# dwofk/fast-depth

Hardware: NVIDIA H100
Metric: depth-maps/sec @224x224 b64 (higher is better)
Workload: dtype f16

## Files before the change

### fastdepth_b200/csrc/fd_api.cu

```cuda
#include <algorithm>
#include <cstring>
#include <functional>
#include <string>
#include <vector>

#include "fd_block_plan.h"
#include "fd_conv_plan.h"
#include "fd_common.cuh"

namespace fd {

BlockPlanOut block_tc_debug_plan(int ksize, int stride, int h_out, int w_out, int n, int c_in, int c_out, int head);
ConvPlanOut conv_tc_debug_plan(int kind, int ksize, int h_out, int w_out, int n, int c_in, int c_out, int n_sms);
ConvPlanOut pw_tf32x3_debug_plan(int h_out, int w_out, int n, int c_in, int c_out, int upsample, int n_sms);

static thread_local std::string g_last_error;
void set_error(const std::string& msg) { g_last_error = msg; }
int fail(int code, const std::string& msg) {
    g_last_error = msg;
    return code;
}

int launch_stem(int dtype, const void* x, void* out, const float* w, const float* scale, const float* bias,
                const StageGeom& g, cudaStream_t st);
int launch_dw(int dtype, const BlockArgs& a, cudaStream_t st);
int launch_pw(int dtype, const BlockArgs& a, cudaStream_t st);
int launch_conv(int dtype, const void* in, const void* w, void* out, const float* scale, const float* bias, const StageGeom& g,
                cudaStream_t st);
int launch_convt(int dtype, int kind, const void* in, const void* w, void* out, const float* scale, const float* bias,
                 const StageGeom& g, cudaStream_t st);
int launch_head(int dtype, const void* in, void* out, const float* w, float scale, float bias, long long m_total, int c,
                int in_pitch, int h, int wd, int up, int act, cudaStream_t st);
int launch_metrics(int dtype, const void* pred, const float* target, int n, int hw, double* sums, cudaStream_t st);
int launch_nyu_val_gather(int dtype, const uint8_t* rgb, const float* depth, const int* rows, const int* cols, int n, int h_in,
                          int w_in, int oh, int ow, void* x, float* t, cudaStream_t st);
struct BlockTcPlan;
bool block_tc_supported(int dtype, const StageGeom& g, bool head_fused);
int block_tc_prepare(int dtype, const BlockArgs& a, const float* head_w, float head_scale, float head_bias, int head_act,
                     void* head_out, bool tma_epilogue, const TcLaunchOpts& opts, BlockTcPlan** out);
int block_tc_launch(BlockTcPlan* p, cudaStream_t st, void* head_out);
void block_tc_destroy(BlockTcPlan* p);
const char* block_tc_name(BlockTcPlan* p);
int block_tc_trace(BlockTcPlan* bp, cudaStream_t st, void* head_out, unsigned long long* out_host, int* rows, int* cols);
struct ChainTcPlan;
bool chain_tc_supported(int dtype, const StageGeom* g, int n_layers);
int chain_tc_prepare(int dtype, const BlockArgs* layers, int n_layers, const TcLaunchOpts& opts, ChainTcPlan** out);
int chain_tc_launch(ChainTcPlan* cp, cudaStream_t st);
void chain_tc_destroy(ChainTcPlan* cp);
const char* chain_tc_name(ChainTcPlan* cp);
int chain_tc_trace(ChainTcPlan* cp, cudaStream_t st, unsigned long long* out_host, int* rows, int* cols);
struct StemTcPlan;
bool stem_tc_supported(int dtype, const StageGeom& g);
int stem_tc_prepare(int dtype, const StageGeom& g, const float* w27_dev, const float* scale_dev, const float* bias_dev, void* out,
                    const TcLaunchOpts& opts, StemTcPlan** res);
int stem_tc_launch(StemTcPlan* sp, const void* x, cudaStream_t st);
void stem_tc_destroy(StemTcPlan* sp);
const char* stem_tc_name(StemTcPlan* sp);
struct ConvTcPlan;
bool conv_tc_supported(int dtype, const StageGeom& g, int kind);
int conv_tc_prepare(int dtype, int kind, const StageGeom& g, const void* in, const void* w, const float* scale_dev,
                    const float* bias_dev, void* out, const TcLaunchOpts& opts, ConvTcPlan** res);
int conv_tc_launch(ConvTcPlan* cp, cudaStream_t st);
void conv_tc_destroy(ConvTcPlan* cp);
const char* conv_tc_name(ConvTcPlan* cp);
bool pw_tf32x3_supported(const StageGeom& g);
int pw_tf32x3_prepare(const StageGeom& g, const void* mid, const float* w, const float* scale_dev, const float* bias_dev,
                      void* out, int out_pitch, int reduce, const TcLaunchOpts& opts, ConvTcPlan** res);

static size_t dtype_size(int dtype) { return dtype == FD_F32 ? 4 : 2; }
static bool is_phased(int kind) { return kind == FD_STAGE_DECONV || kind == FD_STAGE_UPCONV; }
static bool is_conv(int kind) { return kind == FD_STAGE_CONV || is_phased(kind); }

struct Stage {
    fd_stage_desc d{};
    StageGeom g{};
    int out_h = 0, out_w = 0;
    void* out = nullptr;
    void* out_eff = nullptr;
    void* out_alloc = nullptr;
    int out_c = 0;
    int out_pitch = 0;
    int concat_src = -1;
    void* mid = nullptr;
    float* dw_w = nullptr;
    float* dw_scale = nullptr;
    float* dw_bias = nullptr;
    void* pw_w = nullptr;
    float* pw_w_f32 = nullptr;
    float* pw_scale = nullptr;
    float* pw_bias = nullptr;
    float head_scale = 0.f, head_bias = 0.f;
    bool have_weights = false;
    BlockTcPlan* tc = nullptr;
    StemTcPlan* stc = nullptr;
    ConvTcPlan* ctc = nullptr;
    ChainTcPlan* chain = nullptr;
    int chained = 0;
};

struct Step {
    int stage;
    std::string name;
    double alg_bytes, macs;
    double dw_macs = 0.0;
    std::function<int(cudaStream_t, const void*, void*)> run;
};

}

using namespace fd;

struct fd_plan {
    int n = 0, h = 0, w = 0, dtype = 0, device = 0, n_sms = 132;
    std::vector<Stage> stages;
    std::vector<Step> steps;
    bool steps_valid = false;
    int opt_path = 1, opt_fold_head = 1, opt_graph = 1, opt_tma_epilogue = 1, opt_inplace_skip = 1, opt_pdl = 0, opt_wait_sleep_ns = 0;
    int opt_chain = 1;
    int opt_cluster = 1;
    int opt_tf32x3 = 0;
    size_t workspace_bytes = 0;
    struct PipeSlot { void* x = nullptr; void* y = nullptr; cudaEvent_t up = nullptr, done = nullptr, down = nullptr; bool busy = false; };
    PipeSlot pipe[3];
    cudaStream_t pipe_h2d = nullptr, pipe_run = nullptr, pipe_d2h = nullptr;
    unsigned long long pipe_next = 0;
    void* stage_x = nullptr;
    void* stage_y = nullptr;
    cudaEvent_t last_done = nullptr;
    cudaStream_t last_stream = nullptr;
    bool last_stream_set = false;
    void* l2_flush = nullptr;
    size_t l2_flush_bytes = 0;
    struct GraphEntry { const void* x; void* y; cudaGraphExec_t exec; unsigned long long stamp; };
    std::vector<GraphEntry> graphs;
    unsigned long long graph_clock = 0;
    int graph_misses = 0;
};
static const size_t kMaxGraphs = 8;

namespace fd {

struct DeviceGuard {
    int prev = -1;
    bool ok = true;
    explicit DeviceGuard(int dev) {
        if (cudaGetDevice(&prev) != cudaSuccess) { ok = false; return; }
        if (prev != dev && cudaSetDevice(dev) != cudaSuccess) ok = false;
    }
    ~DeviceGuard() {
        if (prev >= 0) cudaSetDevice(prev);
    }
};

static int dev_alloc(fd_plan* p, void** ptr, size_t bytes) {
    bytes = (bytes + 255) & ~size_t(255);
    FD_CUDA_OK(cudaMalloc(ptr, bytes));
    FD_CUDA_OK(cudaMemset(*ptr, 0, bytes));
    p->workspace_bytes += bytes;
    return FD_OK;
}

static void invalidate(fd_plan* p) {
    p->steps_valid = false;
    p->steps.clear();
    for (auto& g : p->graphs) cudaGraphExecDestroy(g.exec);
    p->graphs.clear();
    for (auto& s : p->stages) {
        if (s.tc) { block_tc_destroy(s.tc); s.tc = nullptr; }
        if (s.stc) { stem_tc_destroy(s.stc); s.stc = nullptr; }
        if (s.ctc) { conv_tc_destroy(s.ctc); s.ctc = nullptr; }
        if (s.chain) { chain_tc_destroy(s.chain); s.chain = nullptr; }
        s.chained = 0;
    }
}

static int upload_as_dtype(int dtype, const float* host, size_t count, void* dev) {
    if (dtype == FD_F32) {
        FD_CUDA_OK(cudaMemcpy(dev, host, count * 4, cudaMemcpyHostToDevice));
    } else if (dtype == FD_F16) {
        std::vector<__half> tmp(count);
        for (size_t i = 0; i < count; ++i) tmp[i] = __float2half_rn(host[i]);
        FD_CUDA_OK(cudaMemcpy(dev, tmp.data(), count * 2, cudaMemcpyHostToDevice));
    } else {
        std::vector<__nv_bfloat16> tmp(count);
        for (size_t i = 0; i < count; ++i) tmp[i] = __float2bfloat16_rn(host[i]);
        FD_CUDA_OK(cudaMemcpy(dev, tmp.data(), count * 2, cudaMemcpyHostToDevice));
    }
    return FD_OK;
}

static int build_steps(fd_plan* p) {
    invalidate(p);
    const int ns = (int)p->stages.size();
    const double es = (double)dtype_size(p->dtype);
    for (auto& s : p->stages)
        if (!s.have_weights) return fail(FD_ERR_STATE, "fd_plan_set_stage_weights was not called for every stage");

    TcLaunchOpts lopts;
    lopts.pdl = p->opt_pdl; lopts.sleep_ns = p->opt_wait_sleep_ns; lopts.n_sms = p->n_sms; lopts.cluster = p->opt_cluster;
    Stage& head = p->stages[ns - 1];
    Stage& last = p->stages[ns - 2];
    const bool fold = p->opt_fold_head && (last.d.kind == FD_STAGE_DWPW || last.d.kind == FD_STAGE_CONV) && last.d.upsample &&
                      last.d.skip_src < 0;
    bool head_fused = false;

    for (int i = 0; i < ns; ++i) {
        Stage& s = p->stages[i];
        const void* in = i > 0 ? p->stages[i - 1].out_eff : nullptr;
        s.out_eff = s.out;
        s.g.in_pitch = i > 0 ? p->stages[i - 1].out_pitch : 0;
        s.g.out_pitch = s.out_pitch;
        s.g.skip_pitch = (s.d.skip_src >= 0 && !s.d.skip_mode) ? p->stages[s.d.skip_src].out_pitch : s.out_pitch;
        if (s.d.kind == FD_STAGE_STEM) {
            Step st;
            st.stage = i;
            st.name = "stem_kernel";
            st.macs = (double)s.g.n * s.g.h_out * s.g.w_out * s.g.c_out * 27.0;
            st.alg_bytes = ((double)s.g.n * 3 * s.g.h_in * s.g.w_in + (double)s.g.n * s.g.h_out * s.g.w_out * s.g.c_out) * es +
                           29.0 * s.g.c_out * 4;
            Stage* sp = &s;
            const int dtype = p->dtype;
            if (p->opt_path == 1 && stem_tc_supported(dtype, s.g)) {
                int rc = stem_tc_prepare(dtype, s.g, s.pw_w_f32, s.pw_scale, s.pw_bias, s.out, lopts, &s.stc);
                if (rc != FD_OK) return rc;
                st.name = stem_tc_name(s.stc);
                StemTcPlan* stc = s.stc;
                st.run = [stc](cudaStream_t stream, const void* x, void*) { return stem_tc_launch(stc, x, stream); };
            } else {
                st.run = [sp, dtype](cudaStream_t stream, const void* x, void*) {
                    return launch_stem(dtype, x, sp->out, sp->pw_w_f32, sp->pw_scale, sp->pw_bias, sp->g, stream);
                };
            }
            p->steps.push_back(st);
        } else if (is_conv(s.d.kind)) {
            StageGeom g = s.g;
            if (fold && &s == &last) g.upsample = 0;
            const int kind = s.d.kind;
            const double px_in = (double)g.n * g.h_in * g.w_in, px_out = (double)g.n * g.h_out * g.w_out;
            const double kk = (double)g.ksize * g.ksize;
            Step st;
            st.stage = i;
            st.macs = px_out * g.c_in * g.c_out * kk;
            st.dw_macs = 0.0;
            st.alg_bytes = (px_in * g.c_in + px_out * (g.upsample || is_phased(kind) ? 4.0 : 1.0) * g.c_out) * es +
                           kk * g.c_in * g.c_out * es + 2.0 * g.c_out * 4;
            const int dtype = p->dtype;
            if (p->opt_path == 1 && conv_tc_supported(dtype, g, kind)) {
                int rc = conv_tc_prepare(dtype, kind, g, in, s.pw_w, s.pw_scale, s.pw_bias, s.out, lopts, &s.ctc);
                if (rc != FD_OK) return rc;
                st.name = conv_tc_name(s.ctc);
                ConvTcPlan* ctc = s.ctc;
                st.run = [ctc](cudaStream_t stream, const void*, void*) { return conv_tc_launch(ctc, stream); };
            } else if (kind == FD_STAGE_CONV) {
                char nm[64];
                snprintf(nm, sizeof(nm), "conv_kernel<k%d>", g.ksize);
                st.name = nm;
                Stage* sp = &s;
                st.run = [sp, in, g, dtype](cudaStream_t stream, const void*, void*) {
                    return launch_conv(dtype, in, sp->pw_w, sp->out, sp->pw_scale, sp->pw_bias, g, stream);
                };
            } else {
                char nm[64];
                snprintf(nm, sizeof(nm), "convt_kernel<%s%d>", kind == FD_STAGE_DECONV ? "deconv" : "upconv", g.ksize);
                st.name = nm;
                Stage* sp = &s;
                st.run = [sp, in, g, dtype, kind](cudaStream_t stream, const void*, void*) {
                    return launch_convt(dtype, kind, in, sp->pw_w, sp->out, sp->pw_scale, sp->pw_bias, g, stream);
                };
            }
            p->steps.push_back(st);
        } else if (s.d.kind == FD_STAGE_DWPW && s.chained) {
            continue;
        } else if (s.d.kind == FD_STAGE_DWPW) {
            if (p->opt_path == 1 && p->opt_chain) {
                std::vector<BlockArgs> run;
                std::vector<StageGeom> geoms;
                int j = i;
                for (; j < ns - 1 && (int)run.size() < 8; ++j) {
                    Stage& t = p->stages[j];
                    if (t.d.kind != FD_STAGE_DWPW || t.d.ksize != 3 || t.d.stride != 1 || t.d.upsample || t.d.skip_src >= 0) break;
                    if (j > i && p->stages[j - 1].concat_src >= 0) break;
                    bool is_skip_source = false;
                    for (int k2 = j + 1; k2 < ns; ++k2) if (p->stages[k2].d.skip_src == j) is_skip_source = true;
                    BlockArgs b{};
                    b.g = t.g;
                    b.g.in_pitch = j > 0 ? p->stages[j - 1].out_pitch : 0;
                    b.g.out_pitch = t.out_pitch;
                    b.in = j > 0 ? p->stages[j - 1].out_eff : nullptr;
                    b.out = t.out;
                    b.dw_w = t.dw_w; b.dw_scale = t.dw_scale; b.dw_bias = t.dw_bias;
                    b.pw_w = t.pw_w; b.pw_scale = t.pw_scale; b.pw_bias = t.pw_bias;
                    run.push_back(b); geoms.push_back(b.g);
                    if (is_skip_source) { ++j; break; }
                }
                int len = (int)run.size();
                while (len >= 2 && !chain_tc_supported(p->dtype, geoms.data(), len)) --len;
                if (len >= 2) {
                    int rc = chain_tc_prepare(p->dtype, run.data(), len, lopts, &s.chain);
                    if (rc != FD_OK) return rc;
                    Step st;
                    st.stage = i + len - 1;
                    st.macs = 0; st.dw_macs = 0;
                    double wb = 0;
                    for (int k2 = 0; k2 < len; ++k2) {
                        const StageGeom& g = geoms[k2];
                        const double px = (double)g.n * g.h_out * g.w_out;
                        st.dw_macs += px * g.c_in * 9.0;
                        st.macs += px * g.c_in * 9.0 + px * g.c_in * g.c_out;
                        wb += (double)g.c_in * 9 * 4 + 2.0 * g.c_in * 4 + (double)g.c_in * g.c_out * es + 2.0 * g.c_out * 4;
                        p->stages[i + k2].chained = 1;
                        p->stages[i + k2].out_eff = p->stages[i + k2].out;
                    }
                    st.alg_bytes = ((double)geoms[0].n * geoms[0].h_in * geoms[0].w_in * geoms[0].c_in +
                                    (double)geoms[len - 1].n * geoms[len - 1].h_out * geoms[len - 1].w_out * geoms[len - 1].c_out) * es + wb;
                    char nm[200];
                    snprintf(nm, sizeof(nm), "%s{stages %d-%d}", chain_tc_name(s.chain), i, i + len - 1);
                    st.name = nm;
                    ChainTcPlan* cpn = s.chain;
                    st.run = [cpn](cudaStream_t stream, const void*, void*) { return chain_tc_launch(cpn, stream); };
                    p->steps.push_back(st);
                    s.chained = 1;
                    continue;
                }
            }
            BlockArgs a{};
            a.g = s.g;
            const bool folded_here = fold && (&s == &last);
            if (folded_here) a.g.upsample = 0;
            a.in = in;
            a.mid = s.mid;
            a.out = s.out;
            a.skip = (s.d.skip_src >= 0 && !s.d.skip_mode) ? p->stages[s.d.skip_src].out_eff : nullptr;
            a.dw_w = s.dw_w; a.dw_scale = s.dw_scale; a.dw_bias = s.dw_bias;
            a.pw_w = s.pw_w; a.pw_scale = s.pw_scale; a.pw_bias = s.pw_bias;
            const double px_in = (double)s.g.n * s.g.h_in * s.g.w_in, px_out = (double)s.g.n * s.g.h_out * s.g.w_out;
            const double up = a.g.upsample ? 4.0 : 1.0;
            const double dw_macs = px_out * s.g.c_in * s.g.ksize * s.g.ksize, pw_macs = px_out * s.g.c_in * s.g.c_out;
            const double w_bytes = (double)s.g.c_in * s.g.ksize * s.g.ksize * 4 + 2.0 * s.g.c_in * 4 +
                                   (double)s.g.c_in * s.g.c_out * es + 2.0 * s.g.c_out * 4;
            const double fused_bytes = (px_in * s.g.c_in + px_out * up * s.g.c_out * (a.skip ? 2.0 : 1.0)) * es + w_bytes;
            const int dtype = p->dtype;
            const bool fuse_head = folded_here && p->opt_path == 1 && block_tc_supported(dtype, a.g, true);
            bool use_tc = p->opt_path == 1 && block_tc_supported(dtype, a.g, false);
            if (use_tc) {
                const bool tma_epi = p->opt_tma_epilogue != 0;
                if (tma_epi && p->opt_inplace_skip && a.skip != nullptr) { a.out = const_cast<void*>(a.skip); s.out_eff = a.out; }
                int rc = fuse_head ? block_tc_prepare(dtype, a, head.pw_w_f32, head.head_scale, head.head_bias, head.g.act, nullptr, false, lopts, &s.tc)
                                   : block_tc_prepare(dtype, a, nullptr, 0.f, 0.f, 0, nullptr, tma_epi && (a.skip == nullptr || a.skip == a.out), lopts, &s.tc);
                if (rc != FD_OK) return rc;
                Step st;
                st.stage = i;
                st.name = block_tc_name(s.tc);
                st.macs = dw_macs + pw_macs + (fuse_head ? px_out * s.g.c_out : 0.0);
                st.dw_macs = dw_macs;
                st.alg_bytes = fuse_head ? (px_in * s.g.c_in + px_out * 4.0) * es + w_bytes + s.g.c_out * 4.0 : fused_bytes;
                BlockTcPlan* tc = s.tc;
                st.run = [tc](cudaStream_t stream, const void*, void* y) { return block_tc_launch(tc, stream, y); };
                p->steps.push_back(st);
                head_fused = fuse_head;
            } else {
                Step d;
                d.stage = i;
                d.name = s.g.ksize == 3 ? "dw_kernel<3>" : "dw_kernel<5>";
                d.macs = dw_macs;
                d.dw_macs = dw_macs;
                d.alg_bytes = (px_in + px_out) * s.g.c_in * es + (double)s.g.c_in * (s.g.ksize * s.g.ksize + 2) * 4;
                d.run = [a, dtype](cudaStream_t stream, const void*, void*) { return launch_dw(dtype, a, stream); };
                p->steps.push_back(d);
                Step q;
                q.stage = i;
                q.name = "pw_kernel";
                q.macs = pw_macs;
                q.alg_bytes = (px_out * s.g.c_in + px_out * up * s.g.c_out * (a.skip ? 2.0 : 1.0)) * es +
                              (double)s.g.c_in * s.g.c_out * es + 2.0 * s.g.c_out * 4;
                if (dtype == FD_F32 && p->opt_path == 1 && p->opt_tf32x3 && pw_tf32x3_supported(a.g)) {
                    const bool add = a.skip != nullptr;
                    const bool inplace = add && p->opt_inplace_skip;
                    void* out = inplace ? const_cast<void*>(a.skip) : a.out;
                    const int opitch = inplace ? a.g.skip_pitch : a.g.out_pitch;
                    if (inplace) s.out_eff = out;
                    int rc = pw_tf32x3_prepare(a.g, a.mid, static_cast<const float*>(a.pw_w), a.pw_scale, a.pw_bias, out, opitch,
                                               add ? 1 : 0, lopts, &s.ctc);
                    if (rc != FD_OK) return rc;
                    q.name = conv_tc_name(s.ctc);
                    ConvTcPlan* ctc = s.ctc;
                    const bool copy = add && !inplace;
                    const void* skip = a.skip;
                    const size_t rows = (size_t)a.g.n * s.out_h * s.out_w, row_bytes = (size_t)a.g.c_out * 4;
                    const size_t dpitch = (size_t)a.g.out_pitch * 4, spitch = (size_t)a.g.skip_pitch * 4;
                    q.run = [ctc, copy, out, skip, rows, row_bytes, dpitch, spitch](cudaStream_t stream, const void*, void*) {
                        if (copy)
                            FD_CUDA_OK(cudaMemcpy2DAsync(out, dpitch, skip, spitch, row_bytes, rows, cudaMemcpyDeviceToDevice, stream));
                        return conv_tc_launch(ctc, stream);
                    };
                } else {
                    q.run = [a, dtype](cudaStream_t stream, const void*, void*) { return launch_pw(dtype, a, stream); };
                }
                p->steps.push_back(q);
            }
        } else if (!head_fused) {
            const bool up = fold;
            const int hh = up ? last.g.h_out : s.g.h_in, ww = up ? last.g.w_out : s.g.w_in;
            const long long m_total = (long long)s.g.n * hh * ww;
            Step st;
            st.stage = i;
            st.name = up ? "head_kernel<up2x>" : "head_kernel";
            st.macs = (double)m_total * s.g.c_in;
            st.alg_bytes = ((double)m_total * s.g.c_in + (double)s.g.n * s.g.h_in * s.g.w_in) * es + s.g.c_in * 4.0;
            Stage* sp = &s;
            const int dtype = p->dtype;
            const int c = s.g.c_in, act = s.g.act, ipitch = s.g.in_pitch;
            st.run = [sp, in, dtype, m_total, c, ipitch, hh, ww, up, act](cudaStream_t stream, const void*, void* y) {
                return launch_head(dtype, in, y, sp->pw_w_f32, sp->head_scale, sp->head_bias, m_total, c, ipitch, hh, ww, up ? 1 : 0,
                                   act, stream);
            };
            p->steps.push_back(st);
        }
    }
    p->steps_valid = true;
    return FD_OK;
}

static int run_steps(fd_plan* p, const void* x, void* y, cudaStream_t st) {
    for (auto& s : p->steps) {
        int rc = s.run(st, x, y);
        if (rc != FD_OK) return fail(rc, std::string(fd_last_error()) + " [stage " + std::to_string(s.stage) + ": " + s.name + "]");
    }
    return FD_OK;
}

}

extern "C" {

int fd_abi_version(void) { return FD_ABI_VERSION; }
const char* fd_last_error(void) { return g_last_error.c_str(); }

int fd_plan_create(const fd_stage_desc* stages, int n_stages, int n, int h, int w, int dtype, int device, fd_plan** out) {
    if (!out) return fail(FD_ERR_INVALID, "out is NULL");
    *out = nullptr;
    if (!stages || n_stages < 3) return fail(FD_ERR_INVALID, "need at least stem + one block + head");
    if (n <= 0 || h <= 0 || w <= 0) return fail(FD_ERR_INVALID, "n, h, w must be positive");
    if (h % 32 || w % 32) return fail(FD_ERR_INVALID, "H and W must be multiples of 32 (skip shapes would not line up)");
    if (dtype != FD_F32 && dtype != FD_F16 && dtype != FD_BF16) return fail(FD_ERR_INVALID, "bad dtype");
    int ndev = 0;
    if (cudaGetDeviceCount(&ndev) != cudaSuccess || ndev == 0)
        return fail(FD_ERR_CUDA, "no CUDA device: fastdepth_b200 has no CPU fallback");
    if (device < 0 || device >= ndev) return fail(FD_ERR_INVALID, "bad device index");
    cudaDeviceProp prop{};
    FD_CUDA_OK(cudaGetDeviceProperties(&prop, device));
    if (prop.major != 9 || prop.minor != 0) return fail(FD_ERR_UNSUPPORTED, "fastdepth_b200 is built for sm_90a (H100) only");
    DeviceGuard guard(device);
    if (!guard.ok) return fail(FD_ERR_CUDA, "cudaSetDevice failed");

    fd_plan* p = new fd_plan();
    p->n = n; p->h = h; p->w = w; p->dtype = dtype; p->device = device; p->n_sms = prop.multiProcessorCount;
    p->stages.resize(n_stages);
    const size_t es = dtype_size(dtype);
    int ch = 3, hh = h, ww = w;
    int rc = FD_OK;
    for (int i = 0; i < n_stages && rc == FD_OK; ++i) {
        Stage& s = p->stages[i];
        s.d = stages[i];
        const fd_stage_desc& d = s.d;
        const bool first = i == 0, lastst = i == n_stages - 1;
        if ((d.kind == FD_STAGE_STEM) != first || (d.kind == FD_STAGE_HEAD) != lastst ||
            (!first && !lastst && d.kind != FD_STAGE_DWPW && !is_conv(d.kind))) {
            rc = fail(FD_ERR_INVALID, "stage list must be STEM, (DWPW|CONV|DECONV|UPCONV)..., HEAD"); break; }
        if (d.c_in != ch) { rc = fail(FD_ERR_INVALID, "stage " + std::to_string(i) + ": c_in does not match producer"); break; }
        if (d.act != FD_ACT_RELU && d.act != FD_ACT_RELU6) { rc = fail(FD_ERR_INVALID, "bad act"); break; }
        s.g.n = n; s.g.h_in = hh; s.g.w_in = ww; s.g.c_in = d.c_in; s.g.c_out = d.c_out;
        s.g.ksize = d.ksize; s.g.stride = d.stride; s.g.act = d.act; s.g.upsample = d.upsample ? 1 : 0;
        if (d.kind == FD_STAGE_STEM) {
            if (d.ksize != 3 || d.c_in != 3 || d.c_out % 8 || d.stride < 1 || d.stride > 2 || d.upsample || d.skip_src >= 0) {
                rc = fail(FD_ERR_INVALID, "stem must be 3x3, c_in 3, c_out % 8 == 0, stride 1|2"); break; }
            s.g.h_out = (hh + 2 - 3) / d.stride + 1; s.g.w_out = (ww + 2 - 3) / d.stride + 1;
        } else if (d.kind == FD_STAGE_DWPW) {
            if ((d.ksize != 3 && d.ksize != 5) || d.stride < 1 || d.stride > 2 || d.c_in % 8 || d.c_out % 8 || d.c_out <= 0) {
                rc = fail(FD_ERR_INVALID, "block stage needs k in {3,5}, stride 1|2, channels % 8 == 0"); break; }
            const int pad = (d.ksize - 1) / 2;
            s.g.h_out = (hh + 2 * pad - d.ksize) / d.stride + 1; s.g.w_out = (ww + 2 * pad - d.ksize) / d.stride + 1;
        } else if (d.kind == FD_STAGE_CONV) {
            if (d.skip_src >= 0) { rc = fail(FD_ERR_INVALID, "stage " + std::to_string(i) + ": a CONV stage takes no skip"); break; }
            if (d.stride != 1) { rc = fail(FD_ERR_INVALID, "stage " + std::to_string(i) + ": a CONV stage has stride 1"); break; }
            if ((d.ksize != 3 && d.ksize != 5) || d.c_in % 8 || d.c_out % 8 || d.c_out <= 0 || (d.upsample != 0 && d.upsample != 1)) {
                rc = fail(FD_ERR_INVALID, "conv stage needs k in {3,5}, channels % 8 == 0, upsample 0|1"); break; }
            s.g.h_out = hh; s.g.w_out = ww;
        } else if (is_phased(d.kind)) {
            const char* nm = d.kind == FD_STAGE_DECONV ? "a DECONV" : "an UPCONV";
            if (d.skip_src >= 0) { rc = fail(FD_ERR_INVALID, "stage " + std::to_string(i) + ": " + nm + " stage takes no skip"); break; }
            if (d.stride != 2) { rc = fail(FD_ERR_INVALID, "stage " + std::to_string(i) + ": " + nm + " stage has stride 2"); break; }
            if (d.upsample != 0) { rc = fail(FD_ERR_INVALID, "stage " + std::to_string(i) + ": " + nm + " stage has upsample 0"); break; }
            const bool k_ok = d.kind == FD_STAGE_DECONV ? (d.ksize == 3 || d.ksize == 5 || d.ksize == 7 || d.ksize == 9) : d.ksize == 5;
            if (!k_ok || d.c_in % 8 || d.c_out % 8 || d.c_out <= 0) {
                rc = fail(FD_ERR_INVALID, d.kind == FD_STAGE_DECONV ? "deconv stage needs k in {3,5,7,9}, channels % 8 == 0"
                                                                    : "upconv stage needs k 5, channels % 8 == 0");
                break; }
            s.g.h_out = hh; s.g.w_out = ww;
        } else {
            if (d.ksize != 1 || d.c_out != 1 || d.c_in % 8 || d.upsample || d.skip_src >= 0) {
                rc = fail(FD_ERR_INVALID, "head must be 1x1, c_out 1, c_in % 8 == 0"); break; }
            s.g.h_out = hh; s.g.w_out = ww;
        }
        s.out_h = s.g.h_out * (s.g.upsample || is_phased(d.kind) ? 2 : 1);
        s.out_w = s.g.w_out * (s.g.upsample || is_phased(d.kind) ? 2 : 1);
        s.out_c = d.c_out; s.out_pitch = d.c_out;
        if (d.skip_src >= 0) {
            if (d.kind != FD_STAGE_DWPW || !d.upsample || d.skip_src >= i) { rc = fail(FD_ERR_INVALID, "bad skip_src"); break; }
            Stage& src = p->stages[d.skip_src];
            if (src.out_h != s.out_h || src.out_w != s.out_w || (!d.skip_mode && src.g.c_out != d.c_out)) {
                rc = fail(FD_ERR_INVALID, "stage " + std::to_string(i) + ": skip tensor shape does not match the upsampled output");
                break; }
            if (d.skip_mode) {
                if (d.skip_mode != 1 || src.concat_src >= 0 || src.d.skip_src >= 0) { rc = fail(FD_ERR_INVALID, "bad skip_mode / skip source"); break; }
                s.out_c = d.c_out + src.g.c_out; s.out_pitch = s.out_c;
            }
        }
        if (d.kind != FD_STAGE_HEAD) {
            rc = dev_alloc(p, &s.out, (size_t)n * s.out_h * s.out_w * s.out_pitch * es);
            if (rc) break;
            s.out_alloc = s.out;
            if (d.skip_src >= 0 && d.skip_mode) {
                Stage& src = p->stages[d.skip_src];
                src.out = static_cast<char*>(s.out) + (size_t)d.c_out * es;
                src.out_pitch = s.out_pitch;
                src.concat_src = i;
            }
        }
        if (d.kind == FD_STAGE_DWPW) {
            if ((rc = dev_alloc(p, &s.mid, (size_t)n * s.g.h_out * s.g.w_out * d.c_in * es))) break;
            if ((rc = dev_alloc(p, (void**)&s.dw_w, (size_t)d.ksize * d.ksize * d.c_in * 4))) break;
            if ((rc = dev_alloc(p, (void**)&s.dw_scale, (size_t)d.c_in * 4))) break;
            if ((rc = dev_alloc(p, (void**)&s.dw_bias, (size_t)d.c_in * 4))) break;
            if ((rc = dev_alloc(p, &s.pw_w, (size_t)d.c_in * d.c_out * es))) break;
        } else if (is_conv(d.kind)) {
            if ((rc = dev_alloc(p, &s.pw_w, (size_t)d.ksize * d.ksize * d.c_in * d.c_out * es))) break;
        } else if (d.kind == FD_STAGE_STEM) {
            if ((rc = dev_alloc(p, (void**)&s.pw_w_f32, (size_t)27 * d.c_out * 4))) break;
        } else {
            if ((rc = dev_alloc(p, (void**)&s.pw_w_f32, (size_t)d.c_in * 4))) break;
        }
        if ((rc = dev_alloc(p, (void**)&s.pw_scale, (size_t)d.c_out * 4))) break;
        if ((rc = dev_alloc(p, (void**)&s.pw_bias, (size_t)d.c_out * 4))) break;
        ch = s.out_c; hh = s.out_h; ww = s.out_w;
    }
    if (rc == FD_OK && (hh != h || ww != w)) rc = fail(FD_ERR_INVALID, "stage list does not return to the input resolution");
    if (rc != FD_OK) {
        std::string keep = g_last_error;
        fd_plan_destroy(p);
        g_last_error = keep;
        return rc;
    }
    *out = p;
    return FD_OK;
}

int fd_plan_set_stage_weights(fd_plan* p, int stage, const float* dw_w, const float* dw_scale, const float* dw_bias,
                              const float* pw_w, const float* pw_scale, const float* pw_bias) {
    if (!p) return fail(FD_ERR_INVALID, "plan is NULL");
    if (stage < 0 || stage >= (int)p->stages.size()) return fail(FD_ERR_INVALID, "bad stage index");
    if (!pw_w || !pw_scale || !pw_bias) return fail(FD_ERR_INVALID, "pw_w / pw_scale / pw_bias are required");
    DeviceGuard guard(p->device);
    Stage& s = p->stages[stage];
    const fd_stage_desc& d = s.d;
    if (d.kind == FD_STAGE_DWPW) {
        if (!dw_w || !dw_scale || !dw_bias) return fail(FD_ERR_INVALID, "block stage needs dw_w / dw_scale / dw_bias");
        const int kk = d.ksize * d.ksize;
        std::vector<float> t((size_t)kk * d.c_in);
        for (int c = 0; c < d.c_in; ++c)
            for (int j = 0; j < kk; ++j) t[(size_t)j * d.c_in + c] = dw_w[(size_t)c * kk + j];
        FD_CUDA_OK(cudaMemcpy(s.dw_w, t.data(), t.size() * 4, cudaMemcpyHostToDevice));
        FD_CUDA_OK(cudaMemcpy(s.dw_scale, dw_scale, (size_t)d.c_in * 4, cudaMemcpyHostToDevice));
        FD_CUDA_OK(cudaMemcpy(s.dw_bias, dw_bias, (size_t)d.c_in * 4, cudaMemcpyHostToDevice));
        int rc = upload_as_dtype(p->dtype, pw_w, (size_t)d.c_in * d.c_out, s.pw_w);
        if (rc) return rc;
    } else if (d.kind == FD_STAGE_CONV) {
        const int kk = d.ksize * d.ksize;
        std::vector<float> t((size_t)d.c_out * kk * d.c_in);
        for (int co = 0; co < d.c_out; ++co)
            for (int ci = 0; ci < d.c_in; ++ci)
                for (int j = 0; j < kk; ++j) t[((size_t)co * kk + j) * d.c_in + ci] = pw_w[((size_t)co * d.c_in + ci) * kk + j];
        int rc = upload_as_dtype(p->dtype, t.data(), t.size(), s.pw_w);
        if (rc) return rc;
    } else if (is_phased(d.kind)) {
        const int k = d.ksize, kk = k * k;
        ConvPhase ph[4];
        conv_phases(d.kind, k, ph);
        std::vector<float> t((size_t)d.c_out * kk * d.c_in);
        for (int q = 0; q < 4; ++q)
            for (int iy = 0; iy < ph[q].ny; ++iy)
                for (int ix = 0; ix < ph[q].nx; ++ix) {
                    const int tap = ph[q].tap0 + iy * ph[q].nx + ix;
                    const int wy = convt_tap(d.kind, k, q >> 1, ph[q].dy0 + iy), wx = convt_tap(d.kind, k, q & 1, ph[q].dx0 + ix);
                    for (int co = 0; co < d.c_out; ++co)
                        for (int ci = 0; ci < d.c_in; ++ci) {
                            const size_t src = d.kind == FD_STAGE_DECONV ? ((size_t)ci * d.c_out + co) * kk : ((size_t)co * d.c_in + ci) * kk;
                            t[((size_t)co * kk + tap) * d.c_in + ci] = pw_w[src + wy * k + wx];
                        }
                }
        int rc = upload_as_dtype(p->dtype, t.data(), t.size(), s.pw_w);
        if (rc) return rc;
    } else if (d.kind == FD_STAGE_STEM) {
        std::vector<float> t((size_t)27 * d.c_out);
        for (int co = 0; co < d.c_out; ++co)
            for (int j = 0; j < 27; ++j) t[(size_t)j * d.c_out + co] = pw_w[(size_t)co * 27 + j];
        FD_CUDA_OK(cudaMemcpy(s.pw_w_f32, t.data(), t.size() * 4, cudaMemcpyHostToDevice));
    } else {
        FD_CUDA_OK(cudaMemcpy(s.pw_w_f32, pw_w, (size_t)d.c_in * 4, cudaMemcpyHostToDevice));
        s.head_scale = pw_scale[0];
        s.head_bias = pw_bias[0];
    }
    FD_CUDA_OK(cudaMemcpy(s.pw_scale, pw_scale, (size_t)d.c_out * 4, cudaMemcpyHostToDevice));
    FD_CUDA_OK(cudaMemcpy(s.pw_bias, pw_bias, (size_t)d.c_out * 4, cudaMemcpyHostToDevice));
    s.have_weights = true;
    invalidate(p);
    return FD_OK;
}

static int* option_slot(fd_plan* p, const char* name) {
    if (!p || !name) return nullptr;
    if (!strcmp(name, "path")) return &p->opt_path;
    if (!strcmp(name, "fold_head")) return &p->opt_fold_head;
    if (!strcmp(name, "graph")) return &p->opt_graph;
    if (!strcmp(name, "tma_epilogue")) return &p->opt_tma_epilogue;
    if (!strcmp(name, "inplace_skip")) return &p->opt_inplace_skip;
    if (!strcmp(name, "pdl")) return &p->opt_pdl;
    if (!strcmp(name, "wait_sleep_ns")) return &p->opt_wait_sleep_ns;
    if (!strcmp(name, "chain")) return &p->opt_chain;
    if (!strcmp(name, "cluster")) return &p->opt_cluster;
    if (!strcmp(name, "tf32x3")) return &p->opt_tf32x3;
    return nullptr;
}

int fd_plan_set_option(fd_plan* p, const char* name, int value) {
    int* slot = option_slot(p, name);
    if (!slot) return fail(FD_ERR_INVALID, std::string("unknown option: ") + (name ? name : "(null)"));
    const bool is_time = !strcmp(name, "wait_sleep_ns");
    if (is_time ? (value < 0 || value > 100000) : (value != 0 && value != 1))
        return fail(FD_ERR_INVALID, is_time ? "wait_sleep_ns must be in [0, 100000]" : "option value must be 0 or 1");
    if (*slot != value) { *slot = value; invalidate(p); }
    return FD_OK;
}

int fd_plan_get_option(fd_plan* p, const char* name, int* value) {
    int* slot = option_slot(p, name);
    if (!slot || !value) return fail(FD_ERR_INVALID, "unknown option or NULL value");
    *value = *slot;
    return FD_OK;
}

static int ensure_steps(fd_plan* p) {
    if (p->steps_valid) return FD_OK;
    return build_steps(p);
}

static int forward_enqueue(fd_plan* p, const void* x_dev, void* y_dev, cudaStream_t st);

int fd_forward(fd_plan* p, const void* x_dev, void* y_dev, void* stream) {
    if (!p || !x_dev || !y_dev) return fail(FD_ERR_INVALID, "NULL argument");
    DeviceGuard guard(p->device);
    int rc = ensure_steps(p);
    if (rc) return rc;
    cudaStream_t st = (cudaStream_t)stream;
    if (!p->last_done) FD_CUDA_OK(cudaEventCreateWithFlags(&p->last_done, cudaEventDisableTiming));
    if (p->last_stream_set && p->last_stream != st) FD_CUDA_OK(cudaStreamWaitEvent(st, p->last_done, 0));
    rc = forward_enqueue(p, x_dev, y_dev, st);
    if (rc) return rc;
    cudaStreamCaptureStatus cs = cudaStreamCaptureStatusNone;
    if (cudaStreamIsCapturing(st, &cs) == cudaSuccess && cs == cudaStreamCaptureStatusNone) {
        FD_CUDA_OK(cudaEventRecord(p->last_done, st));
        p->last_stream = st; p->last_stream_set = true;
    }
    return FD_OK;
}

static int forward_enqueue(fd_plan* p, const void* x_dev, void* y_dev, cudaStream_t st) {
    int rc = FD_OK;
    if (!p->opt_graph) return run_steps(p, x_dev, y_dev, st);

    for (auto& g : p->graphs)
        if (g.x == x_dev && g.y == y_dev) {
            g.stamp = ++p->graph_clock;
            p->graph_misses = 0;
            FD_CUDA_OK(cudaGraphLaunch(g.exec, st));
            return FD_OK;
        }
    if (++p->graph_misses > 2 * (int)kMaxGraphs) {
        if (p->graph_misses > (1 << 30)) p->graph_misses = 2 * (int)kMaxGraphs + 1;
        return run_steps(p, x_dev, y_dev, st);
    }
    cudaStream_t cap;
    FD_CUDA_OK(cudaStreamCreateWithFlags(&cap, cudaStreamNonBlocking));
    cudaGraph_t graph = nullptr;
    cudaGraphExec_t exec = nullptr;
    cudaError_t e = cudaStreamBeginCapture(cap, cudaStreamCaptureModeThreadLocal);
    if (e == cudaSuccess) {
        rc = run_steps(p, x_dev, y_dev, cap);
        e = cudaStreamEndCapture(cap, &graph);
        if (rc == FD_OK && e == cudaSuccess) e = cudaGraphInstantiate(&exec, graph, 0);
    }
    if (graph) cudaGraphDestroy(graph);
    cudaStreamDestroy(cap);
    if (rc != FD_OK) return rc;
    if (e != cudaSuccess) return fail(FD_ERR_CUDA, std::string("graph capture: ") + cudaGetErrorString(e));
    if (p->graphs.size() >= kMaxGraphs) {
        size_t victim = 0;
        for (size_t i = 1; i < p->graphs.size(); ++i)
            if (p->graphs[i].stamp < p->graphs[victim].stamp) victim = i;
        cudaGraphExecDestroy(p->graphs[victim].exec);
        p->graphs.erase(p->graphs.begin() + victim);
    }
    p->graphs.push_back({x_dev, y_dev, exec, ++p->graph_clock});
    FD_CUDA_OK(cudaGraphLaunch(exec, st));
    return FD_OK;
}

int fd_forward_host(fd_plan* p, const void* x_host, void* y_host, void* stream) {
    if (!p || !x_host || !y_host) return fail(FD_ERR_INVALID, "NULL argument");
    DeviceGuard guard(p->device);
    const size_t es = dtype_size(p->dtype);
    const size_t xb = (size_t)p->n * 3 * p->h * p->w * es, yb = (size_t)p->n * p->h * p->w * es;
    if (!p->stage_x) {
        int rc = dev_alloc(p, &p->stage_x, xb);
        if (rc) return rc;
        if ((rc = dev_alloc(p, &p->stage_y, yb))) return rc;
    }
    cudaStream_t st = (cudaStream_t)stream;
    FD_CUDA_OK(cudaMemcpyAsync(p->stage_x, x_host, xb, cudaMemcpyHostToDevice, st));
    int rc = fd_forward(p, p->stage_x, p->stage_y, stream);
    if (rc) return rc;
    FD_CUDA_OK(cudaMemcpyAsync(y_host, p->stage_y, yb, cudaMemcpyDeviceToHost, st));
    FD_CUDA_OK(cudaStreamSynchronize(st));
    return FD_OK;
}

static const int kPipeSlots = 3;

int fd_pipeline_submit(fd_plan* p, const void* x_host, void* y_host, unsigned long long* ticket) {
    if (!p || !x_host || !y_host || !ticket) return fail(FD_ERR_INVALID, "NULL argument");
    DeviceGuard guard(p->device);
    const size_t es = dtype_size(p->dtype);
    const size_t xb = (size_t)p->n * 3 * p->h * p->w * es, yb = (size_t)p->n * p->h * p->w * es;
    if (!p->pipe_h2d) {
        FD_CUDA_OK(cudaStreamCreateWithFlags(&p->pipe_h2d, cudaStreamNonBlocking));
        FD_CUDA_OK(cudaStreamCreateWithFlags(&p->pipe_run, cudaStreamNonBlocking));
        FD_CUDA_OK(cudaStreamCreateWithFlags(&p->pipe_d2h, cudaStreamNonBlocking));
        for (auto& sl : p->pipe) {
            int rc = dev_alloc(p, &sl.x, xb);
            if (rc) return rc;
            if ((rc = dev_alloc(p, &sl.y, yb))) return rc;
            FD_CUDA_OK(cudaEventCreateWithFlags(&sl.up, cudaEventDisableTiming));
            FD_CUDA_OK(cudaEventCreateWithFlags(&sl.done, cudaEventDisableTiming));
            FD_CUDA_OK(cudaEventCreateWithFlags(&sl.down, cudaEventDisableTiming));
        }
    }
    const unsigned long long t = p->pipe_next;
    fd_plan::PipeSlot& sl = p->pipe[t % kPipeSlots];
    if (sl.busy) {
        FD_CUDA_OK(cudaEventSynchronize(sl.down));
        sl.busy = false;
    }
    FD_CUDA_OK(cudaMemcpyAsync(sl.x, x_host, xb, cudaMemcpyHostToDevice, p->pipe_h2d));
    FD_CUDA_OK(cudaEventRecord(sl.up, p->pipe_h2d));
    FD_CUDA_OK(cudaStreamWaitEvent(p->pipe_run, sl.up, 0));
    int rc = fd_forward(p, sl.x, sl.y, p->pipe_run);
    if (rc) return rc;
    FD_CUDA_OK(cudaEventRecord(sl.done, p->pipe_run));
    FD_CUDA_OK(cudaStreamWaitEvent(p->pipe_d2h, sl.done, 0));
    FD_CUDA_OK(cudaMemcpyAsync(y_host, sl.y, yb, cudaMemcpyDeviceToHost, p->pipe_d2h));
    FD_CUDA_OK(cudaEventRecord(sl.down, p->pipe_d2h));
    sl.busy = true;
    *ticket = t;
    p->pipe_next = t + 1;
    return FD_OK;
}

int fd_pipeline_wait(fd_plan* p, unsigned long long ticket) {
    if (!p) return fail(FD_ERR_INVALID, "NULL plan");
    if (ticket >= p->pipe_next) return fail(FD_ERR_INVALID, "unknown ticket");
    if (ticket + kPipeSlots < p->pipe_next) return FD_OK;
    DeviceGuard guard(p->device);
    fd_plan::PipeSlot& sl = p->pipe[ticket % kPipeSlots];
    if (sl.busy) {
        FD_CUDA_OK(cudaEventSynchronize(sl.down));
        sl.busy = false;
    }
    return FD_OK;
}

int fd_stage_buffer(fd_plan* p, int stage, int which, void** dev_ptr, int* n, int* h, int* w, int* c, int* c_stride) {
    if (!p || stage < 0 || stage >= (int)p->stages.size() || !dev_ptr) return fail(FD_ERR_INVALID, "bad argument");
    Stage& s = p->stages[stage];
    int hh, ww, cc;
    void* ptr;
    if (which == 0) {
        ptr = s.out_eff ? s.out_eff : s.out; hh = s.out_h; ww = s.out_w; cc = s.g.c_out;
        if (p->opt_fold_head && stage == (int)p->stages.size() - 2 && s.d.upsample && s.d.skip_src < 0) { hh = s.g.h_out; ww = s.g.w_out; }
    } else if (which == 1) {
        if (is_conv(s.d.kind)) return fail(FD_ERR_INVALID, "a CONV / DECONV / UPCONV stage has no depthwise intermediate");
        ptr = s.mid; hh = s.g.h_out; ww = s.g.w_out; cc = s.g.c_in;
    } else {
        return fail(FD_ERR_INVALID, "which must be 0 or 1");
    }
    if (!ptr) return fail(FD_ERR_STATE, "stage has no such buffer");
    *dev_ptr = ptr;
    if (n) *n = p->n;
    if (h) *h = hh;
    if (w) *w = ww;
    if (c) *c = cc;
    if (c_stride) *c_stride = (which == 0 && s.out_pitch > 0) ? s.out_pitch : cc;
    return FD_OK;
}

int fd_plan_launches_per_forward(fd_plan* p, int* n_launches) {
    if (!p || !n_launches) return fail(FD_ERR_INVALID, "NULL argument");
    DeviceGuard guard(p->device);
    int rc = ensure_steps(p);
    if (rc) return rc;
    *n_launches = (int)p->steps.size();
    return FD_OK;
}

int fd_plan_workspace_bytes(fd_plan* p, size_t* bytes) {
    if (!p || !bytes) return fail(FD_ERR_INVALID, "NULL argument");
    *bytes = p->workspace_bytes;
    return FD_OK;
}

int fd_plan_step_count(fd_plan* p, int* n_steps) { return fd_plan_launches_per_forward(p, n_steps); }

int fd_plan_step_info(fd_plan* p, int step, int* stage, double* alg_bytes, double* macs, char* kernel_name, int name_cap) {
    if (!p) return fail(FD_ERR_INVALID, "NULL plan");
    DeviceGuard guard(p->device);
    int rc = ensure_steps(p);
    if (rc) return rc;
    if (step < 0 || step >= (int)p->steps.size()) return fail(FD_ERR_INVALID, "bad step index");
    const Step& s = p->steps[step];
    if (stage) *stage = s.stage;
    if (alg_bytes) *alg_bytes = s.alg_bytes;
    if (macs) *macs = s.macs;
    if (kernel_name && name_cap > 0) {
        strncpy(kernel_name, s.name.c_str(), name_cap - 1);
        kernel_name[name_cap - 1] = 0;
    }
    return FD_OK;
}

int fd_plan_step_macs(fd_plan* p, int step, double* dw_macs, double* dense_macs) {
    if (!p) return fail(FD_ERR_INVALID, "NULL plan");
    DeviceGuard guard(p->device);
    int rc = ensure_steps(p);
    if (rc) return rc;
    if (step < 0 || step >= (int)p->steps.size()) return fail(FD_ERR_INVALID, "bad step index");
    const Step& s = p->steps[step];
    if (dw_macs) *dw_macs = s.dw_macs;
    if (dense_macs) *dense_macs = s.macs - s.dw_macs;
    return FD_OK;
}

int fd_plan_time_steps(fd_plan* p, const void* x_dev, void* y_dev, void* stream, int warmup, int iters, int flush_l2,
                       float* ms_out) {
    if (!p || !x_dev || !y_dev || !ms_out || iters <= 0) return fail(FD_ERR_INVALID, "bad argument");
    DeviceGuard guard(p->device);
    int rc = ensure_steps(p);
    if (rc) return rc;
    cudaStream_t st = (cudaStream_t)stream;
    if (flush_l2 && !p->l2_flush) {
        p->l2_flush_bytes = size_t(256) << 20;
        FD_CUDA_OK(cudaMalloc(&p->l2_flush, p->l2_flush_bytes));
    }
    rc = run_steps(p, x_dev, y_dev, st);
    if (rc) return rc;
    cudaEvent_t e0, e1;
    FD_CUDA_OK(cudaEventCreate(&e0));
    FD_CUDA_OK(cudaEventCreate(&e1));
    for (size_t i = 0; i < p->steps.size() && rc == FD_OK; ++i) {
        for (int k = 0; k < warmup && rc == FD_OK; ++k) rc = p->steps[i].run(st, x_dev, y_dev);
        float total = 0.f;
        for (int k = 0; k < iters && rc == FD_OK; ++k) {
            if (flush_l2) cudaMemsetAsync(p->l2_flush, k & 0xff, p->l2_flush_bytes, st);
            cudaEventRecord(e0, st);
            rc = p->steps[i].run(st, x_dev, y_dev);
            cudaEventRecord(e1, st);
            cudaError_t e = cudaEventSynchronize(e1);
            if (e != cudaSuccess) { rc = fail(FD_ERR_CUDA, std::string("step ") + p->steps[i].name + ": " + cudaGetErrorString(e)); break; }
            float ms = 0.f;
            cudaEventElapsedTime(&ms, e0, e1);
            total += ms;
        }
        ms_out[i] = total / iters;
    }
    cudaEventDestroy(e0);
    cudaEventDestroy(e1);
    return rc;
}

int fd_plan_trace_stage(fd_plan* p, int stage, void* y_dev, void* stream, unsigned long long* out_host, int cap, int* rows, int* cols) {
    if (!p || stage < 0 || stage >= (int)p->stages.size() || !out_host || !rows || !cols) return fail(FD_ERR_INVALID, "bad argument");
    DeviceGuard guard(p->device);
    int rc = ensure_steps(p);
    if (rc) return rc;
    if (cap < 12 * 256) return fail(FD_ERR_INVALID, "trace buffer too small (need 3072 entries)");
    if (is_conv(p->stages[stage].d.kind)) return fail(FD_ERR_INVALID, "the stage timeline exists for fused block kernels only");
    if (p->stages[stage].chain) return chain_tc_trace(p->stages[stage].chain, (cudaStream_t)stream, out_host, rows, cols);
    if (!p->stages[stage].tc) return fail(FD_ERR_STATE, "stage does not run the fused block kernel");
    return block_tc_trace(p->stages[stage].tc, (cudaStream_t)stream, y_dev, out_host, rows, cols);
}

int fd_debug_block_plan(int ksize, int stride, int h_out, int w_out, int n, int c_in, int c_out, int head, int* out, int cap) {
    if (!out || cap < 16) return fail(FD_ERR_INVALID, "need an int[16] output");
    const BlockPlanOut q = block_tc_debug_plan(ksize, stride, h_out, w_out, n, c_in, c_out, head);
    const int v[16] = {q.ok, q.splits, q.n_cta, q.items, q.kblocks, q.s_in, q.s_a, q.s_b, q.bn, q.nb, q.b_resident, q.n_stg,
                       q.smem_bytes, q.in_stage_stride, q.cs, q.dw_teams};
    for (int i = 0; i < 16; ++i) out[i] = v[i];
    return FD_OK;
}

int fd_debug_conv_plan(int ksize, int h_out, int w_out, int n, int c_in, int c_out, int n_sms, int* out, int cap) {
    if (!out || cap < 16) return fail(FD_ERR_INVALID, "need an int[16] output");
    const ConvPlanOut q = conv_tc_debug_plan(FD_STAGE_CONV, ksize, h_out, w_out, n, c_in, c_out, n_sms);
    const int v[16] = {q.ok, q.ni, q.th, q.tw, q.bn, q.stages, q.m_tiles, q.n_splits, q.items, q.waves, q.kblocks, q.smem_bytes,
                       q.useful_permille, (int)(q.cost > 2e9 ? 2e9 : q.cost), 0, 0};
    for (int i = 0; i < 16; ++i) out[i] = v[i];
    return FD_OK;
}

int fd_debug_pw_tf32x3_plan(int h_out, int w_out, int n, int c_in, int c_out, int upsample, int n_sms, int* out, int cap) {
    if (!out || cap < 16) return fail(FD_ERR_INVALID, "need an int[16] output");
    const ConvPlanOut q = pw_tf32x3_debug_plan(h_out, w_out, n, c_in, c_out, upsample, n_sms);
    const int v[16] = {q.ok, q.ni, q.th, q.tw, q.bn, q.stages, q.m_tiles, q.n_splits, q.items, q.waves, q.kblocks, q.smem_bytes,
                       q.useful_permille, (int)(q.cost > 2e9 ? 2e9 : q.cost), q.ok ? conv_stage_bytes_tf32x3(q.bn) : 0, 0};
    for (int i = 0; i < 16; ++i) out[i] = v[i];
    return FD_OK;
}

int fd_debug_convt_plan(int kind, int ksize, int h_in, int w_in, int n, int c_in, int c_out, int n_sms, int* out, int cap) {
    if (!out || cap < 44) return fail(FD_ERR_INVALID, "need an int[44] output");
    if (!is_phased(kind)) return fail(FD_ERR_INVALID, "kind must be FD_STAGE_DECONV or FD_STAGE_UPCONV");
    const ConvPlanOut q = conv_tc_debug_plan(kind, ksize, h_in, w_in, n, c_in, c_out, n_sms);
    const int v[16] = {q.ok, q.ni, q.th, q.tw, q.bn, q.stages, q.m_tiles, q.n_splits, q.items, q.waves, q.kblocks, q.smem_bytes,
                       q.useful_permille, (int)(q.cost > 2e9 ? 2e9 : q.cost), q.groups, 0};
    for (int i = 0; i < 16; ++i) out[i] = v[i];
    for (int ph = 0; ph < 4; ++ph) {
        const int e[5] = {q.ph[ph].tap0, q.ph[ph].ny, q.ph[ph].nx, q.ph[ph].dy0, q.ph[ph].dx0};
        for (int j = 0; j < 5; ++j) out[16 + 5 * ph + j] = q.ok ? e[j] : 0;
    }
    for (int g = 0; g < 4; ++g)
        for (int j = 0; j < 2; ++j) out[36 + 2 * g + j] = q.ok ? q.group_ph[g][j] : -1;
    return FD_OK;
}

int fd_metrics_accumulate(const void* pred_dev, const float* target_dev, int dtype, int n, int hw, double* sums_dev,
                          int device, void* stream) {
    if (!pred_dev || !target_dev || !sums_dev || n < 0 || hw <= 0) return fail(FD_ERR_INVALID, "bad argument");
    DeviceGuard guard(device);
    if (!guard.ok) return fail(FD_ERR_CUDA, "cudaSetDevice failed");
    return launch_metrics(dtype, pred_dev, target_dev, n, hw, sums_dev, (cudaStream_t)stream);
}

int fd_nyu_val_gather(const uint8_t* rgb_dev, const float* depth_dev, const int* rows_dev, const int* cols_dev, int n, int h_in,
                      int w_in, int out_h, int out_w, int dtype, void* x_dev, float* target_dev, int device, void* stream) {
    if (!rgb_dev || !rows_dev || !cols_dev || !x_dev || n < 0 || h_in <= 0 || w_in <= 0 || out_h <= 0 || out_w <= 0)
        return fail(FD_ERR_INVALID, "bad argument");
    if ((depth_dev == nullptr) != (target_dev == nullptr)) return fail(FD_ERR_INVALID, "depth and target must come together");
    DeviceGuard guard(device);
    if (!guard.ok) return fail(FD_ERR_CUDA, "cudaSetDevice failed");
    return launch_nyu_val_gather(dtype, rgb_dev, depth_dev, rows_dev, cols_dev, n, h_in, w_in, out_h, out_w, x_dev, target_dev,
                                 (cudaStream_t)stream);
}

void fd_plan_destroy(fd_plan* p) {
    if (!p) return;
    DeviceGuard guard(p->device);
    invalidate(p);
    for (auto& s : p->stages) {
        cudaFree(s.out_alloc ? s.out_alloc : s.out); cudaFree(s.mid); cudaFree(s.dw_w); cudaFree(s.dw_scale); cudaFree(s.dw_bias);
        cudaFree(s.pw_w); cudaFree(s.pw_w_f32); cudaFree(s.pw_scale); cudaFree(s.pw_bias);
    }
    for (auto& sl : p->pipe) {
        cudaFree(sl.x); cudaFree(sl.y);
        if (sl.up) cudaEventDestroy(sl.up);
        if (sl.done) cudaEventDestroy(sl.done);
        if (sl.down) cudaEventDestroy(sl.down);
    }
    if (p->last_done) cudaEventDestroy(p->last_done);
    if (p->pipe_h2d) cudaStreamDestroy(p->pipe_h2d);
    if (p->pipe_run) cudaStreamDestroy(p->pipe_run);
    if (p->pipe_d2h) cudaStreamDestroy(p->pipe_d2h);
    cudaFree(p->stage_x); cudaFree(p->stage_y); cudaFree(p->l2_flush);
    delete p;
}

}
```

### fastdepth_b200/csrc/fd_block_plan.h

```cpp
#pragma once

namespace fd {

constexpr int kPlanKblk = 64;
constexpr int kPlanAStage = 128 * 128;
constexpr int kPlanStg = 16384;
constexpr int kPlanMaxIn = 6, kPlanMaxA = 4, kPlanMaxB = 16;
constexpr int kPlanMaxACluster = 6;
constexpr int kPlanMaxNcta = 128;
#ifdef __CUDACC__
__host__ __device__
#endif
constexpr int dw_taps_bytes(int ksize) { return ksize == 5 ? 5 * 32 * 48 : ksize * ksize * 64 * 2; }
#ifndef FD_PLAN_SMALL_SMEM
constexpr int kPlanSmemBudget = 227 * 1024 - 128;
constexpr int kPlanAlignSlack = 1024;
#else
constexpr int kPlanSmemBudget = 224 * 1024;
constexpr int kPlanAlignSlack = 2048;
#endif

struct BlockPlanIn {
    int ksize, stride, tile;
    int c_in, c_out, n_tiles;
    int head;
    int barrier_bytes;
    int max_n_cta;
    int n_sms;
    int even_rings;
    int cluster_multiwave;
    int cluster;
};
struct BlockPlanOut {
    int ok;
    int kblocks, cin_pad, splits, n_cta, cpad_all, items;
    int in_stage_bytes, dwp_bytes, in_stage_stride;
    int s_in, s_a, s_b, bn, nb, b_resident, b_stage_bytes;
    int n_stg;
    int dw_teams;
    int cs;
    int smem_bytes;
};

inline bool plan_block_smem(const BlockPlanIn& q, BlockPlanOut& p) {
    const int splits = p.splits;
    const int sms = q.n_sms > 0 ? q.n_sms : 132;
    const int fixed = q.barrier_bytes + kPlanAlignSlack + (q.head ? 3 : 2) * p.cpad_all * 4;
    const int total = kPlanSmemBudget - fixed;
    long best = -(1L << 60);
    bool found = false;
    const int bn_top = (p.n_cta + 63) / 64 * 64;
    const int per_cta_kb = p.cs > 1 ? (p.kblocks + p.cs - 1) / p.cs : p.kblocks;
    for (int s_a = p.cs > 1 ? kPlanMaxACluster : kPlanMaxA; s_a >= 2; --s_a)
        for (int n_stg = q.head ? 0 : 2; n_stg >= (q.head ? 0 : 1); --n_stg) {
            if (q.even_rings == 1 && p.cs == 1 && (s_a & 1)) continue;
            const int avail = total - s_a * kPlanAStage - n_stg * kPlanStg;
            for (int bn = bn_top; bn >= 64; bn -= 64) {
                const int nb = (p.n_cta + bn - 1) / bn;
                const int w_all = p.kblocks * nb * bn * 128;
                const bool can_res = splits == 1 && bn == bn_top && p.kblocks * nb <= kPlanMaxB && w_all <= 64 * 1024;
                for (int res = can_res ? 1 : 0; res >= 0; --res)
                    for (int s_b = res ? p.kblocks * nb : 6; s_b >= (res ? p.kblocks * nb : 2); --s_b) {
                        if (!res && s_b > p.kblocks * nb && s_b > 2) continue;
                        const int left = avail - s_b * bn * 128;
                        if (left < 0) continue;
                        int s_in = left / p.in_stage_stride;
                        if (s_in > kPlanMaxIn) s_in = kPlanMaxIn;
                        if (q.even_rings == 1 && p.cs == 1 && s_in >= 2) s_in &= ~1;
                        if (q.even_rings && p.cs == 1 && s_in > 4) s_in &= ~1;
                        if (s_in < 2 && !(s_in == 1 && p.kblocks == 1 && p.items <= sms)) continue;
                        if (p.cs > 1 && s_in > per_cta_kb + 1) s_in = per_cta_kb + 1 < 2 ? 2 : per_cta_kb + 1;
                        const int b_ahead2 = res ? 4 : (2 * s_b / nb > 4 ? 4 : 2 * s_b / nb);
                        long score = (long)bn * 100 + (s_in > 4 ? 4 : s_in) * 2500 + s_a * (p.kblocks <= 2 ? 1500 : 400) + n_stg * 2800 +
                                     (res ? 1000 : 0) + b_ahead2 * 1800;
                        if (p.cs > 1)
                            score = (long)bn * 100 + (s_in > 3 ? 3 : s_in) * 1500 + (s_a > p.cs + 1 ? p.cs + 1 : s_a) * 4000 + n_stg * 2800 +
                                    b_ahead2 * 2500;
                        if (score > best) {
                            found = true; best = score;
                            p.s_a = s_a; p.n_stg = n_stg; p.s_in = s_in; p.s_b = s_b; p.bn = bn; p.b_resident = res;
                        }
                    }
            }
        }
    if (!found) return false;
    p.nb = (p.n_cta + p.bn - 1) / p.bn;
    p.b_stage_bytes = p.bn * 128;
    p.smem_bytes = p.s_a * kPlanAStage + p.s_b * p.b_stage_bytes + p.s_in * p.in_stage_stride + p.n_stg * kPlanStg + fixed;
    return true;
}

inline int plan_dw_teams(const BlockPlanIn& q, const BlockPlanOut& p) {
    return (q.even_rings && p.cs == 1 && p.s_in >= 2 && !(p.s_in & 1) && !(p.s_a & 1) && (q.even_rings == 1 || p.kblocks == 1)) ? 2 : 1;
}

inline BlockPlanOut plan_block(const BlockPlanIn& q) {
    BlockPlanOut p{};
    const long sms = q.n_sms > 0 ? q.n_sms : 132;
    const int NI = q.tile ? 2 : 1, TH = 8, TW = q.tile ? 8 : 16;
    const int IH = (TH - 1) * q.stride + q.ksize, IW = (TW - 1) * q.stride + q.ksize;
    p.kblocks = (q.c_in + kPlanKblk - 1) / kPlanKblk;
    p.cin_pad = p.kblocks * kPlanKblk;
    p.in_stage_bytes = NI * IH * IW * 128;
    p.dwp_bytes = dw_taps_bytes(q.ksize) + 512;
    p.in_stage_stride = (p.in_stage_bytes + p.dwp_bytes + 127) / 128 * 128;
    const int cout_pad = (q.c_out + 15) / 16 * 16;
    struct Cand { long t; int sp, nc, cs; };
    Cand cands[12];
    int n_cands = 0;
    if (cout_pad <= 64 || q.head) {
        cands[n_cands++] = Cand{0, 1, cout_pad, 1};
    } else {
        const long dw_c = 2L * q.ksize * q.ksize * 64;
        for (int n_cta = kPlanMaxNcta; n_cta >= 64; n_cta -= 64) {
            int sp = (cout_pad + n_cta - 1) / n_cta, nc = n_cta;
            if (sp == 1) nc = cout_pad;
            if (sp == 1 && cout_pad > kPlanMaxNcta) continue;
            if (sp == 1 && n_cta - 64 >= cout_pad) continue;
            if (q.max_n_cta > 0 && nc > q.max_n_cta && !(sp == 1 && cout_pad <= kPlanMaxNcta)) continue;
            const long items = (long)q.n_tiles * sp;
            const long rounds = (items + sms - 1) / sms;
            const long active = items < sms ? items : sms;
            const long mma_c = 4L * nc;
            const long l2_c = active * (p.in_stage_bytes + 128L * nc) / 3000;
            long kb_c = dw_c > mma_c ? dw_c : mma_c;
            if (l2_c > kb_c) kb_c = l2_c;
            const long t = rounds * (p.kblocks * (kb_c + 100) + 8L * nc);
            int at = n_cands++;
            while (at > 0 && cands[at - 1].t > t) { cands[at] = cands[at - 1]; --at; }
            cands[at] = Cand{t, sp, nc, 1};
        }
        for (int cs = 2; cs <= 4 && q.cluster != 1; cs *= 2) {
            if (q.cluster > 1 && q.cluster != cs) continue;
            if (q.cluster == 0 && !(q.ksize == 5 && q.tile == 1 && cs == 4)) continue;
            if ((long)q.n_tiles * cs > sms && !q.cluster_multiwave) continue;
            const int nc = ((cout_pad + cs - 1) / cs + 63) / 64 * 64;
            if (nc > kPlanMaxNcta || nc * (cs - 1) >= cout_pad || p.kblocks < cs) continue;
            const long n_cl = sms / cs;
            const long rounds = ((long)q.n_tiles + n_cl - 1) / n_cl;
            const long mma_c = 4L * nc;
            const long active = (q.n_tiles < n_cl ? q.n_tiles : n_cl) * cs;
            const long l2_c = active * (p.in_stage_bytes / cs + 128L * nc) / 3000;
            long kb_c = dw_c / cs > mma_c ? dw_c / cs : mma_c;
            if (l2_c > kb_c) kb_c = l2_c;
            long t = rounds * (p.kblocks * (kb_c + 150) + 8L * nc) + 1500;
            if (q.cluster > 1) t = -1;
            int at = n_cands++;
            while (at > 0 && cands[at - 1].t > t) { cands[at] = cands[at - 1]; --at; }
            cands[at] = Cand{t, cs, nc, cs};
        }
    }
    for (int i = 0; i < n_cands; ++i) {
        p.splits = cands[i].sp; p.n_cta = cands[i].nc; p.cs = cands[i].cs;
        p.items = q.n_tiles * p.splits;
        p.cpad_all = p.n_cta * p.splits;
        if (plan_block_smem(q, p)) { p.ok = 1; p.dw_teams = plan_dw_teams(q, p); return p; }
    }
    p.ok = 0;
    return p;
}

}
```

### fastdepth_b200/csrc/fd_block_tc.cu

```cuda
#include <cuda.h>

#include <cstdio>
#include <cstdlib>
#include <cstring>
#include <new>
#include <string>

#include "fd_block_plan.h"
#include "fd_tc_common.cuh"

namespace fd {

constexpr int TC_DW_WARPS = 8;
constexpr int TC_EPI_WARPS = 8;
constexpr int TC_WARP_EPI0 = 0, TC_WARP_DW0 = TC_EPI_WARPS;
constexpr int TC_WARP_TMA = TC_DW_WARPS + TC_EPI_WARPS;
constexpr int TC_THREADS = (TC_WARP_TMA + 1) * 32;
constexpr int TC_WARP_BCAST = TC_WARP_TMA + 1;
constexpr int TC_THREADS_CL = (TC_WARP_BCAST + 1) * 32;
constexpr int TC_NCH = 2;
constexpr int TC_KBLK = 64;
constexpr int TC_A_STAGE_BYTES = 128 * 128;
constexpr int TC_MAX_IN = 6, TC_MAX_A = 6, TC_MAX_B = 16;
static_assert(TC_MAX_A >= kPlanMaxACluster && TC_MAX_A >= kPlanMaxA && TC_MAX_IN >= kPlanMaxIn && TC_MAX_B >= kPlanMaxB, "barrier arrays cover the planner's ring depths");
constexpr int TC_TRACE_N = 256;

struct TcParams {
    int n, h_in, w_in, h_out, w_out, c_in, c_out;
    int tiles_x, tiles_y;
    int items, splits;
    int kblocks;
    int cin_pad;
    int n_cta;
    int bn;
    int nb;
    int s_in, s_a, s_b;
    int b_resident;
    int in_stage_bytes, b_stage_bytes;
    int act, upsample;
    int head;
    int head_act;
    float head_scale, head_bias;
    const void* skip;
    void* out;
    void* head_out;
    int in_stage_stride;
    int dwp_bytes;
    int cpad_all;
    int n_stg;
    int out_pitch, skip_pitch;
    int sleep_ns;
    int mma_sleep_ns;
    int dw_sleep_ns;
    int epi_tma;
    int epi_red;
    unsigned long long mg_splits, mg_tx, mg_ty;
    const void* dwp;
    const float2* pw_affine;
    const float* head_w;
    int dw_teams;
    int epi_high;
    int wmc;
    int cs;
    unsigned long long* trace;
};

struct TcBarriers {
    uint64_t in_full[TC_MAX_IN], in_empty[TC_MAX_IN];
    uint64_t a_full[TC_MAX_A], a_empty[TC_MAX_A];
    uint64_t b_full[TC_MAX_B], b_empty[TC_MAX_B];
    uint64_t aff_full;
    uint64_t dw_done[4];
};

struct ItemCoord { int img0, oy0, ox0, n0; };
__device__ __forceinline__ ItemCoord decode_item(const TcParams& p, int w, int NI, int TH, int TW) {
    ItemCoord c;
    uint32_t t = fdiv40((uint32_t)w, p.mg_splits);
    const int split = w - (int)t * p.splits;
    uint32_t t2 = fdiv40(t, p.mg_tx);
    const int tile_x = (int)(t - t2 * (uint32_t)p.tiles_x);
    uint32_t t3 = fdiv40(t2, p.mg_ty);
    const int tile_y = (int)(t2 - t3 * (uint32_t)p.tiles_y);
    c.img0 = (int)t3 * NI; c.oy0 = tile_y * TH; c.ox0 = tile_x * TW; c.n0 = split * p.n_cta;
    return c;
}

#define TC_TRACE(row, idx)                                                                       \
    do {                                                                                         \
        if (p.trace != nullptr && blockIdx.x == 0 && (idx) < TC_TRACE_N) p.trace[(row) * TC_TRACE_N + (idx)] = clock64(); \
    } while (0)

template <typename T, int KS, int STRIDE, int NI, int TH, int TW, bool RELU6, bool HALFK = false, int CLM = 0>
__global__ void __launch_bounds__(CLM == 1 ? TC_THREADS_CL : TC_THREADS, 1)
block_tc_kernel(const __grid_constant__ CUtensorMap tm_in, const __grid_constant__ CUtensorMap tm_w,
                const __grid_constant__ CUtensorMap tm_o0, const __grid_constant__ CUtensorMap tm_o1,
                const __grid_constant__ CUtensorMap tm_o2, const __grid_constant__ CUtensorMap tm_o3, const TcParams p) {
    static_assert(NI * TH * TW == 128, "tile must hold 128 pixels");
    static_assert(NI * (TH / 4) * (TW / 4) == TC_DW_WARPS, "one 4x4 pixel block per depthwise warp");
    constexpr int PAD = (KS - 1) / 2;
    constexpr int IH = (TH - 1) * STRIDE + KS, IW = (TW - 1) * STRIDE + KS;
    constexpr int IBH = 3 * STRIDE + KS, IBW = 3 * STRIDE + KS;
    using MF = MixFma<T>;

    extern __shared__ uint8_t smem_raw[];
    const uint32_t smem_base = (smem_u32(smem_raw) + 1023u) & ~1023u;
    uint8_t* smem = smem_raw + (smem_base - smem_u32(smem_raw));
    const uint32_t a_off = 0;
    const uint32_t b_off = a_off + p.s_a * TC_A_STAGE_BYTES;
    const uint32_t stg_off = b_off + p.s_b * p.b_stage_bytes;
    const uint32_t in_off = stg_off + (uint32_t)p.n_stg * 16384u;
    const uint32_t pw_off = in_off + p.s_in * p.in_stage_stride;
    const uint32_t bar_off = pw_off + (p.head ? 3u : 2u) * (uint32_t)p.cpad_all * 4u;
    TcBarriers* bars = reinterpret_cast<TcBarriers*>(smem + bar_off);
    float2* s_pw_affine = reinterpret_cast<float2*>(smem + pw_off);
    uint32_t* s_head_w2 = reinterpret_cast<uint32_t*>(s_pw_affine + p.cpad_all);

    const int warp = threadIdx.x >> 5, lane = threadIdx.x & 31;
    const int rwarp = (p.epi_high && warp < TC_DW_WARPS + TC_EPI_WARPS) ? (warp ^ 8) : warp;
    constexpr bool CL = CLM == 1, CW = CLM == 2;
    constexpr bool kHint = CLM != 1;
    static_assert(!(HALFK && CLM != 0), "the half-K block has one K-block and resident weights: nothing to share");
    const uint32_t cs = CL ? (uint32_t)p.cs : 1u;
    const uint32_t crank = (CL || CW) ? cluster_ctarank() : 0u;
    const uint32_t wmc = CW ? (uint32_t)p.wmc : 1u;
    const int u_first = CW ? (int)(blockIdx.x / wmc) : (int)blockIdx.x;
    const int u_stride = CW ? (int)(gridDim.x / wmc) : (int)gridDim.x;
    const int u_count = CW ? p.items / (int)wmc : p.items;
    auto item_of = [&](int u) -> int {
        if (!CW) return u;
        const int g = (int)fdiv40((uint32_t)u, p.mg_splits), sp = u - g * p.splits;
        return (g * (int)wmc + (int)crank) * p.splits + sp;
    };

    if (threadIdx.x == 0) {
        const uint32_t dw_arrivals = (uint32_t)(TC_DW_WARPS / ((CL || p.dw_teams != 2) ? 1 : 2));
        for (int i = 0; i < TC_MAX_IN; ++i) { mbar_init(smem_u32(&bars->in_full[i]), 1); mbar_init(smem_u32(&bars->in_empty[i]), dw_arrivals); }
        for (int i = 0; i < TC_MAX_A; ++i) { mbar_init(smem_u32(&bars->a_full[i]), CL ? 1u : dw_arrivals); mbar_init(smem_u32(&bars->a_empty[i]), 2u * cs); }
        for (int i = 0; i < 4; ++i) mbar_init(smem_u32(&bars->dw_done[i]), TC_DW_WARPS);
        for (int i = 0; i < TC_MAX_B; ++i) { mbar_init(smem_u32(&bars->b_full[i]), 1); mbar_init(smem_u32(&bars->b_empty[i]), 2u * wmc); }
        mbar_init(smem_u32(&bars->aff_full), 1);
        fence_barrier_init();
        mbar_expect_tx(smem_u32(&bars->aff_full), (uint32_t)p.cpad_all * 8u);
        bulk_load(smem_base + pw_off, p.pw_affine, (uint32_t)p.cpad_all * 8u, smem_u32(&bars->aff_full));
    }
#ifdef FD_TC_WATCHDOG_MAP
    if (blockIdx.x == 0 && threadIdx.x == 0)
        printf("WATCHDOG map (cs %d wmc %d items %d kb %d s_in %d s_a %d s_b %d): in_full %u in_empty %u a_full %u a_empty %u b_full %u b_empty %u acc_full %u acc_empty %u dw_done %u\n",
               p.cs, p.wmc, p.items, p.kblocks, p.s_in, p.s_a, p.s_b, smem_u32(&bars->in_full[0]), smem_u32(&bars->in_empty[0]), smem_u32(&bars->a_full[0]),
               smem_u32(&bars->a_empty[0]), smem_u32(&bars->b_full[0]), smem_u32(&bars->b_empty[0]), smem_u32(&bars->acc_full[0]), smem_u32(&bars->acc_empty[0]),
               smem_u32(&bars->dw_done[0]));
#endif
    if (warp == TC_WARP_TMA && lane == 0) {
        tma_prefetch_desc(&tm_in);
        tma_prefetch_desc(&tm_w);
        if (p.epi_tma) { tma_prefetch_desc(&tm_o0); if (p.upsample) { tma_prefetch_desc(&tm_o1); tma_prefetch_desc(&tm_o2); tma_prefetch_desc(&tm_o3); } }
    }
    if (p.head)
        for (int i = 2 * threadIdx.x; i < p.cpad_all; i += 2 * (int)blockDim.x) s_head_w2[i >> 1] = MF::pack(p.head_w[i], p.head_w[i + 1]);
    if constexpr (HALFK) {
        for (int i = threadIdx.x; i < p.s_a * (TC_A_STAGE_BYTES / 16); i += (int)blockDim.x)
            reinterpret_cast<uint4*>(smem + a_off)[i] = make_uint4(0u, 0u, 0u, 0u);
        fence_proxy_async();
    }
    pdl_launch_dependents();
    pdl_wait_prior_grid();
    if constexpr (CLM != 0) cluster_sync_all();
    else __syncthreads();

    if (warp == TC_WARP_TMA) {
        if (lane == 0) {
            Ring rin;
            int tr = 0;
            for (int u = u_first; u < u_count; u += u_stride) {
                const int w = item_of(u);
                const ItemCoord c = decode_item(p, w, NI, TH, TW);
                for (int kb = CL ? (int)crank : 0; kb < p.kblocks; kb += (int)cs, rin.next((uint32_t)p.s_in)) {
                    const uint32_t s = rin.s, ph = rin.ph;
                    mbar_wait_sleep_sel<kHint>(smem_u32(&bars->in_empty[s]), ph ^ 1u, (uint32_t)p.sleep_ns >> 2);
                    mbar_expect_tx(smem_u32(&bars->in_full[s]), (uint32_t)(p.in_stage_bytes + p.dwp_bytes));
                    tma_load_4d(smem_base + in_off + s * p.in_stage_stride, &tm_in, smem_u32(&bars->in_full[s]), kb * TC_KBLK,
                                c.ox0 * STRIDE - PAD, c.oy0 * STRIDE - PAD, c.img0);
                    bulk_load(smem_base + in_off + s * p.in_stage_stride + p.in_stage_bytes,
                              reinterpret_cast<const uint8_t*>(p.dwp) + (size_t)kb * p.dwp_bytes, (uint32_t)p.dwp_bytes,
                              smem_u32(&bars->in_full[s]));
                    TC_TRACE(0, tr); ++tr;
                }
            }
        } else if (lane == 1) {
            Ring rb;
            bool first = true;
            const uint16_t w_mask = (uint16_t)((1u << wmc) - 1u);
            const uint32_t slice_rows = (uint32_t)p.bn / wmc, slice_bytes = slice_rows * 128u;
            for (int u = u_first; u < u_count; u += u_stride, first = false) {
                if (p.b_resident && !first) break;
                const int w = item_of(u);
                const int n0 = (w - (int)fdiv40((uint32_t)w, p.mg_splits) * p.splits) * p.n_cta;
                for (int kb = 0; kb < p.kblocks; ++kb)
                    for (int nbi = 0; nbi < p.nb; ++nbi) {
                        uint32_t sb;
                        if (p.b_resident) {
                            sb = (uint32_t)(kb * p.nb + nbi);
                        } else {
                            sb = rb.s;
                            mbar_wait_sleep_sel<kHint>(smem_u32(&bars->b_empty[sb]), rb.ph ^ 1u, (uint32_t)p.sleep_ns >> 2);
                            rb.next((uint32_t)p.s_b);
                        }
                        mbar_expect_tx(smem_u32(&bars->b_full[sb]), (uint32_t)p.b_stage_bytes);
                        if constexpr (CW)
                            tma_load_2d_multicast(smem_base + b_off + sb * p.b_stage_bytes + crank * slice_bytes, &tm_w,
                                                  smem_u32(&bars->b_full[sb]), kb * TC_KBLK, n0 + nbi * p.bn + (int)(crank * slice_rows), w_mask);
                        else
                            tma_load_2d(smem_base + b_off + sb * p.b_stage_bytes, &tm_w, smem_u32(&bars->b_full[sb]), kb * TC_KBLK,
                                        n0 + nbi * p.bn);
                    }
            }
        }
    } else if (CL && warp == TC_WARP_BCAST) {
        if (lane == 0) {
            Ring ra;
            uint32_t o = 0;
            for (int u = u_first; u < u_count; u += u_stride)
                for (int kb = 0; kb < p.kblocks; ++kb, ra.next((uint32_t)p.s_a)) {
                    if ((uint32_t)kb % cs != crank) continue;
                    mbar_wait_sel<kHint>(smem_u32(&bars->dw_done[o & 3u]), (o >> 2) & 1u);
                    ++o;
                    const uint32_t slot = smem_base + a_off + ra.s * TC_A_STAGE_BYTES, bar = smem_u32(&bars->a_full[ra.s]);
                    mbar_arrive(bar);
                    for (uint32_t peer = 0; peer < cs; ++peer)
                        if (peer != crank) bulk_copy_to_peer(mapa_u32(slot, peer), slot, (uint32_t)TC_A_STAGE_BYTES, mapa_u32(bar, peer));
                }
        }
    } else if (rwarp >= TC_WARP_DW0 && rwarp < TC_WARP_DW0 + TC_DW_WARPS) {
        constexpr int BPR = TW / 4, BPI = (TH / 4) * BPR;
        const int dwi = rwarp - TC_WARP_DW0;
        const int teams = CL ? 1 : p.dw_teams;
        const int team = teams == 2 ? dwi >> 2 : 0, member = teams == 2 ? dwi & 3 : dwi, nblk = teams;
        Ring rin, ra;
        int tr = 0;
        uint32_t own = 0;
        const bool tracer = dwi == 0 && lane == 0;
        for (int u = u_first; u < u_count; u += u_stride) {
            for (int kb = 0; kb < p.kblocks; ++kb, ra.next((uint32_t)p.s_a)) {
                if (CL && (uint32_t)kb % cs != crank) {
                    mbar_wait_sel<kHint>(smem_u32(&bars->a_empty[ra.s]), ra.ph ^ 1u);
                    continue;
                }
                const uint32_t s = rin.s, ph = rin.ph, sa = ra.s, pha = ra.ph;
                rin.next((uint32_t)p.s_in);
                if (teams == 2 && (int)(own & 1u) != team) { ++own; continue; }
                mbar_wait_sleep_sel<kHint>(smem_u32(&bars->in_full[s]), ph, (uint32_t)p.dw_sleep_ns);
                if (tracer) TC_TRACE(1, tr);
                const uint8_t* stage = smem + in_off + s * p.in_stage_stride;
                const uint8_t* prm = stage + p.in_stage_bytes;
                constexpr int TAPS = dw_taps_bytes(KS);
                const f32x2 sc = *reinterpret_cast<const f32x2*>(prm + TAPS + lane * 8);
                const f32x2 bi = *reinterpret_cast<const f32x2*>(prm + TAPS + 256 + lane * 8);
                mbar_wait_sel<kHint>(smem_u32(&bars->a_empty[sa]), pha ^ 1u);
                uint8_t* a_s = smem + a_off + sa * TC_A_STAGE_BYTES;
#pragma unroll 1
                for (int blk = 0; blk < nblk; ++blk) {
                const int bidx = member * nblk + blk;
                const int ni = bidx / BPI, rem = bidx % BPI, br = rem / BPR, bc = rem % BPR;
                const uint8_t* in_s = stage + (uint32_t)((ni * IH + br * 4 * STRIDE) * IW + bc * 4 * STRIDE) * 128u + lane * 4u;
                if constexpr (HALFK) {
                    static_assert(KS == 3 && STRIDE == 1, "half-K depthwise exists for the 3x3 stride-1 block only");
                    const int hl = lane & 15, hh = lane >> 4;
                    const uint8_t* in_h = in_s - lane * 4 + hl * 4 + (hh * 2 * IW) * 128;
                    const f32x2 sc2 = *reinterpret_cast<const f32x2*>(prm + TAPS + hl * 8);
                    const f32x2 bi2 = *reinterpret_cast<const f32x2*>(prm + TAPS + 256 + hl * 8);
                    f32x2 acc[2][4];
#pragma unroll
                    for (int a = 0; a < 2; ++a)
#pragma unroll
                        for (int b = 0; b < 4; ++b) acc[a][b] = 0ull;
                    f32x2 wq[KS][KS];
#pragma unroll
                    for (int iy = 0; iy < 1 + KS; ++iy) {
                        if (iy < KS) {
#pragma unroll
                            for (int kx = 0; kx < KS; ++kx)
                                wq[iy][kx] = MF::widen(*reinterpret_cast<const uint32_t*>(prm + (iy * KS + kx) * 128 + hl * 4));
                        }
                        f32x2 row[IBW];
#pragma unroll
                        for (int ix = 0; ix < IBW; ++ix) row[ix] = MF::widen(*reinterpret_cast<const uint32_t*>(in_h + (iy * IW + ix) * 128));
#pragma unroll
                        for (int oy = 0; oy < 2; ++oy) {
                            const int ky = iy - oy;
                            if (ky < 0 || ky >= KS) continue;
#pragma unroll
                            for (int ox = 0; ox < 4; ++ox)
#pragma unroll
                                for (int kx = 0; kx < KS; ++kx) ffma2(acc[oy][ox], row[ox + kx], wq[ky][kx]);
                            if (ky == KS - 1) {
#pragma unroll
                                for (int ox = 0; ox < 4; ++ox) {
                                    const int m = (ni * TH + br * 4 + hh * 2 + oy) * TW + bc * 4 + ox;
                                    *reinterpret_cast<uint32_t*>(a_s + m * 128 + (((hl >> 2) ^ (m & 7)) << 4) + ((hl & 3) << 2)) =
                                        MF::template pack_act<RELU6>(ffma2_abc(acc[oy][ox], sc2, bi2));
                                }
                            }
                        }
                    }
                } else {
                    f32x2 acc[4][4];
#pragma unroll
                    for (int a = 0; a < 4; ++a)
#pragma unroll
                        for (int b = 0; b < 4; ++b) acc[a][b] = 0ull;
                    constexpr bool kTapsInRegs = KS == 3;
                    f32x2 wq[kTapsInRegs ? KS : 1][KS];
#pragma unroll
                    for (int iy = 0; iy < IBH; ++iy) {
                        if constexpr (kTapsInRegs) {
                            if (iy < KS) {
#pragma unroll
                                for (int kx = 0; kx < KS; ++kx)
                                    wq[iy][kx] = MF::widen(*reinterpret_cast<const uint32_t*>(prm + (iy * KS + kx) * 128 + lane * 4));
                            }
                        }
                        f32x2 row[IBW];
#pragma unroll
                        for (int ix = 0; ix < IBW; ++ix) row[ix] = MF::widen(*reinterpret_cast<const uint32_t*>(in_s + (iy * IW + ix) * 128));
#pragma unroll
                        for (int oy = 0; oy < 4; ++oy) {
                            const int ky = iy - oy * STRIDE;
                            if (ky < 0 || ky >= KS) continue;
                            f32x2 wk[KS];
                            if constexpr (kTapsInRegs) {
#pragma unroll
                                for (int kx = 0; kx < KS; ++kx) wk[kx] = wq[ky][kx];
                            } else {
                                const uint8_t* tr = prm + (ky * 32 + lane) * 48;
                                const uint4 t01 = lds_u4_here(tr), t23 = lds_u4_here(tr + 16), t4 = lds_u4_here(tr + 32);
                                wk[0] = ((f32x2)t01.y << 32) | t01.x; wk[1] = ((f32x2)t01.w << 32) | t01.z;
                                wk[2] = ((f32x2)t23.y << 32) | t23.x; wk[3] = ((f32x2)t23.w << 32) | t23.z;
                                wk[4] = ((f32x2)t4.y << 32) | t4.x;
                            }
#pragma unroll
                            for (int ox = 0; ox < 4; ++ox)
#pragma unroll
                                for (int kx = 0; kx < KS; ++kx) ffma2(acc[oy][ox], row[ox * STRIDE + kx], wk[kx]);
                            if (ky == KS - 1) {
#pragma unroll
                                for (int ox = 0; ox < 4; ++ox) {
                                    const int m = (ni * TH + br * 4 + oy) * TW + bc * 4 + ox;
                                    *reinterpret_cast<uint32_t*>(a_s + m * 128 + (((lane >> 2) ^ (m & 7)) << 4) + ((lane & 3) << 2)) =
                                        MF::template pack_act<RELU6>(ffma2_abc(acc[oy][ox], sc, bi));
                                }
                            }
                        }
                    }
                }
                }
                if (tracer) TC_TRACE(2, tr);
                __syncwarp();
                if (lane == 0) mbar_arrive(smem_u32(&bars->in_empty[s]));
                fence_proxy_async();
                __syncwarp();
                if (lane == 0) mbar_arrive(CL ? smem_u32(&bars->dw_done[own & 3u]) : smem_u32(&bars->a_full[sa]));
                ++own;
                if (tracer) { TC_TRACE(3, tr); ++tr; }
            }
        }
    } else {
        const int ew = rwarp - TC_WARP_EPI0;
        const int wg = ew >> 2, wq = ew & 3;
        const int r0 = wg * 64 + wq * 16 + (lane >> 2), cq = (lane & 3) * 2;
        const bool leader = wq == 0 && lane == 0;
        const bool elected = ew == 0 && lane == 0;
        constexpr uint32_t bar_id = 1u, bar_n = 256u;
        T* __restrict__ outp = reinterpret_cast<T*>(p.out);
        const T* __restrict__ skipp = reinterpret_cast<const T*>(p.skip);
        const int n_stg = p.n_stg < 2 ? 1 : 2;
        const int nch = (p.n_cta + 63) >> 6;
        const int bn_ch = p.bn >> 6;
        const uint32_t a_lo0 = sw128_desc_lo(smem_base + a_off + (uint32_t)wg * 8192u), b_lo0 = sw128_desc_lo(smem_base + b_off);
        const uint32_t a_step = TC_A_STAGE_BYTES >> 4, b_step = (uint32_t)p.b_stage_bytes >> 4;
        Ring ra, rb;
        int tr = 0;
        uint32_t stg_flip = 0;
        bool first = true;
        int kb_arm = 0;
        long q_left = 0;
        if constexpr (CL) {
            if (elected) {
                const int n_it = u_first < u_count ? (u_count - 1 - u_first) / u_stride + 1 : 0;
                q_left = (long)n_it * p.kblocks;
                for (int s = 0; s < p.s_a && q_left > 0; ++s, --q_left) {
                    if ((uint32_t)kb_arm % cs != crank) mbar_expect_tx(smem_u32(&bars->a_full[s]), (uint32_t)TC_A_STAGE_BYTES);
                    if (++kb_arm == p.kblocks) kb_arm = 0;
                }
            }
        }
        mbar_wait_sel<kHint>(smem_u32(&bars->aff_full), 0);
        for (int u = u_first; u < u_count; u += u_stride, first = false) {
            const int w = item_of(u);
            const ItemCoord c = decode_item(p, w, NI, TH, TW);
            float acc[TC_NCH][32];
#pragma unroll
            for (int j = 0; j < TC_NCH; ++j)
#pragma unroll
                for (int i = 0; i < 32; ++i) acc[j][i] = 0.f;
            for (int kb = 0; kb < p.kblocks; ++kb, ra.next((uint32_t)p.s_a)) {
                mbar_wait_sleep_sel<kHint>(smem_u32(&bars->a_full[ra.s]), ra.ph, (uint32_t)p.mma_sleep_ns);
                if constexpr (CL) {
                    if (elected && q_left > 0) {
                        if ((uint32_t)kb_arm % cs != crank) mbar_expect_tx(smem_u32(&bars->a_full[ra.s]), (uint32_t)TC_A_STAGE_BYTES);
                        if (++kb_arm == p.kblocks) kb_arm = 0;
                        --q_left;
                    }
                }
                if (elected) TC_TRACE(4, tr);
                uint32_t sbs[TC_NCH] = {0u, 0u};
                for (int nbi = 0; nbi * bn_ch < nch; ++nbi) {
                    uint32_t sb;
                    if (p.b_resident) {
                        sb = (uint32_t)(kb * (nch / bn_ch) + nbi);
                        if (first) mbar_wait_sel<kHint>(smem_u32(&bars->b_full[sb]), 0);
                    } else {
                        sb = rb.s;
                        mbar_wait_sel<kHint>(smem_u32(&bars->b_full[sb]), rb.ph);
                        rb.next((uint32_t)p.s_b);
                    }
                    sbs[nbi] = sb;
                }
                const uint32_t a_lo = a_lo0 + ra.s * a_step;
                wgmma_fence();
#pragma unroll
                for (int j = 0; j < TC_NCH; ++j) {
                    if (j < nch) {
                        const uint32_t b_lo = b_lo0 + (bn_ch == 2 ? sbs[0] * b_step + (uint32_t)j * 512u : sbs[j] * b_step);
#pragma unroll
                        for (int k4 = 0; k4 < 4; ++k4)
                            wgmma_n64<T>(acc[j], sw128_desc(a_lo + 2u * k4), sw128_desc(b_lo + 2u * k4), (kb > 0 || k4 > 0) ? 1u : 0u);
                    }
                }
                wgmma_commit();
                wgmma_wait0();
                if (leader) {
                    const uint32_t bar_a = smem_u32(&bars->a_empty[ra.s]);
                    if constexpr (CL) { for (uint32_t r = 0; r < cs; ++r) mbar_arrive_cluster(mapa_u32(bar_a, r)); }
                    else mbar_arrive(bar_a);
                    if (!p.b_resident)
                        for (int nbi = 0; nbi * bn_ch < nch; ++nbi) {
                            const uint32_t bar_b = smem_u32(&bars->b_empty[sbs[nbi]]);
                            if constexpr (CW) { for (uint32_t r = 0; r < wmc; ++r) mbar_arrive_cluster(mapa_u32(bar_b, r)); }
                            else mbar_arrive(bar_b);
                        }
                }
                if (elected) { TC_TRACE(5, tr); ++tr; }
            }

            if (!p.head) {
                const float2* aff = s_pw_affine + c.n0;
#pragma unroll
                for (int cb = 0; cb < TC_NCH; ++cb) {
                    if (cb >= nch) break;
                    uint8_t* stg = smem + stg_off + (n_stg == 2 ? (stg_flip & 1u) * 16384u : 0u);
                    ++stg_flip;
                    if (n_stg == 1 && stg_flip > 1) {
                        if (p.epi_tma && elected) bulk_wait_read0();
                        asm volatile("bar.sync %0, %1;" ::"r"(bar_id), "r"(bar_n) : "memory");
                    }
#pragma unroll
                    for (int i = 0; i < 8; ++i) {
                        if (cb * 64 + i * 8 < p.n_cta) {
                            const float4 af = *reinterpret_cast<const float4*>(aff + cb * 64 + i * 8 + cq);
                            const f32x2 sc = f32x2_make(af.x, af.y), bi = f32x2_make(af.z, af.w);
#pragma unroll
                            for (int h = 0; h < 2; ++h) {
                                const int r = r0 + 8 * h;
                                *reinterpret_cast<uint32_t*>(stg + r * 128 + ((i ^ (r & 7)) << 4) + cq * 2) =
                                    MF::template pack_act<RELU6>(ffma2_abc(f32x2_make(acc[cb][4 * i + 2 * h], acc[cb][4 * i + 2 * h + 1]), sc, bi));
                            }
                        }
                    }
                    if (p.epi_tma) {
                        fence_proxy_async();
                        if (elected && cb == 0) TC_TRACE(9, tr);
                        if (elected) bulk_wait_read0();
                        asm volatile("bar.sync %0, %1;" ::"r"(bar_id), "r"(bar_n) : "memory");
                        if (elected && cb == 0) TC_TRACE(10, tr);
                        if (elected) {
                            const uint32_t src = smem_u32(stg);
                            const int cc = c.n0 + cb * 64;
                            if (!p.upsample) {
                                tma_store_4d(&tm_o0, src, cc, c.ox0, c.oy0, c.img0);
                            } else if (!p.epi_red) {
                                tma_store_4d(&tm_o0, src, cc, c.ox0, c.oy0, c.img0);
                                tma_store_4d(&tm_o1, src, cc, c.ox0, c.oy0, c.img0);
                                tma_store_4d(&tm_o2, src, cc, c.ox0, c.oy0, c.img0);
                                tma_store_4d(&tm_o3, src, cc, c.ox0, c.oy0, c.img0);
                            } else {
                                tma_reduce_add_4d(&tm_o0, src, cc, c.ox0, c.oy0, c.img0);
                                tma_reduce_add_4d(&tm_o1, src, cc, c.ox0, c.oy0, c.img0);
                                tma_reduce_add_4d(&tm_o2, src, cc, c.ox0, c.oy0, c.img0);
                                tma_reduce_add_4d(&tm_o3, src, cc, c.ox0, c.oy0, c.img0);
                            }
                            bulk_commit_group();
                            if (cb == 0) TC_TRACE(11, tr);
                        }
                        continue;
                    }
                    asm volatile("bar.sync %0, %1;" ::"r"(bar_id), "r"(bar_n) : "memory");
                    const int et = ew * 32 + lane;
                    const int ch = et & 7;
                    const int ccol = cb * 64 + ch * 8;
                    const bool cok = ccol < p.n_cta && c.n0 + ccol + 8 <= p.c_out;
#pragma unroll
                    for (int k = 0; k < 4; ++k) {
                        const int rr = (et >> 3) + 32 * k;
                        const int r_ni = rr / (TH * TW), r_ty = (rr / TW) % TH, r_tx = rr % TW;
                        const int pimg = c.img0 + r_ni, poy = c.oy0 + r_ty, pox = c.ox0 + r_tx;
                        if (!(cok && pimg < p.n && poy < p.h_out && pox < p.w_out)) continue;
                        const uint4 v = *reinterpret_cast<const uint4*>(stg + rr * 128 + ((ch ^ (rr & 7)) << 4));
                        if (!p.upsample) {
                            *reinterpret_cast<uint4*>(outp + (((size_t)pimg * p.h_out + poy) * p.w_out + pox) * p.out_pitch + c.n0 + ccol) = v;
                        } else {
                            const int w2 = 2 * p.w_out;
                            const size_t pix00 = ((size_t)pimg * 2 * p.h_out + 2 * poy) * w2 + 2 * pox;
                            size_t off[4], soff[4];
#pragma unroll
                            for (int d = 0; d < 4; ++d) {
                                const size_t pix = pix00 + (size_t)(d >> 1) * w2 + (d & 1);
                                off[d] = pix * p.out_pitch + c.n0 + ccol;
                                soff[d] = pix * p.skip_pitch + c.n0 + ccol;
                            }
                            if (skipp != nullptr) {
                                uint4 sv[4];
#pragma unroll
                                for (int d = 0; d < 4; ++d) sv[d] = __ldg(reinterpret_cast<const uint4*>(skipp + soff[d]));
                                const uint32_t vv[4] = {v.x, v.y, v.z, v.w};
#pragma unroll
                                for (int d = 0; d < 4; ++d) {
                                    const uint32_t sk[4] = {sv[d].x, sv[d].y, sv[d].z, sv[d].w};
                                    uint32_t z[4];
#pragma unroll
                                    for (int j = 0; j < 4; ++j) {
                                        const float2 a = MF::unpack(vv[j]), bq = MF::unpack(sk[j]);
                                        z[j] = MF::pack(a.x + bq.x, a.y + bq.y);
                                    }
                                    *reinterpret_cast<uint4*>(outp + off[d]) = make_uint4(z[0], z[1], z[2], z[3]);
                                }
                            } else {
#pragma unroll
                                for (int d = 0; d < 4; ++d) *reinterpret_cast<uint4*>(outp + off[d]) = v;
                            }
                        }
                    }
                }
            } else {
                float dot[2][2] = {{0.f, 0.f}, {0.f, 0.f}};
#pragma unroll
                for (int i = 0; i < 8; ++i) {
                    const int c0 = i * 8 + cq;
                    if (i * 8 < p.n_cta) {
                        const float4 af = *reinterpret_cast<const float4*>(s_pw_affine + c0);
                        const f32x2 sc = f32x2_make(af.x, af.y), bi = f32x2_make(af.z, af.w);
                        const uint32_t hw = s_head_w2[c0 >> 1];
#pragma unroll
                        for (int h = 0; h < 2; ++h) {
                            const uint32_t hv = MF::template pack_act<RELU6>(ffma2_abc(f32x2_make(acc[0][4 * i + 2 * h], acc[0][4 * i + 2 * h + 1]), sc, bi));
                            MF::fma2(dot[h][0], dot[h][1], hv, hw);
                        }
                    }
                }
#pragma unroll
                for (int h = 0; h < 2; ++h) {
                    float d = dot[h][0] + dot[h][1];
                    d += __shfl_xor_sync(0xffffffffu, d, 1);
                    d += __shfl_xor_sync(0xffffffffu, d, 2);
                    const int r = r0 + 8 * h;
                    const int img = c.img0 + r / (TH * TW), oy = c.oy0 + (r / TW) % TH, ox = c.ox0 + r % TW;
                    if ((lane & 3) == 0 && img < p.n && oy < p.h_out && ox < p.w_out) {
                        const float y = apply_act(fmaf(d, p.head_scale, p.head_bias), p.head_act);
                        const uint32_t yy = MF::pack(y, y);
                        T* ho = reinterpret_cast<T*>(p.head_out) + ((size_t)img * 2 * p.h_out + 2 * oy) * (2 * p.w_out) + 2 * ox;
                        *reinterpret_cast<uint32_t*>(ho) = yy;
                        *reinterpret_cast<uint32_t*>(ho + 2 * p.w_out) = yy;
                    }
                }
            }
            if (elected) TC_TRACE(7, tr);
        }
        if (p.epi_tma && elected) bulk_wait_all();
    }

    if constexpr (CLM != 0) cluster_sync_all();
}

PFN_encodeTiled get_tensor_map_encoder() {
    static PFN_encodeTiled fn = nullptr;
    if (fn) return fn;
    void* ptr = nullptr;
    cudaDriverEntryPointQueryResult qres;
    if (cudaGetDriverEntryPoint("cuTensorMapEncodeTiled", &ptr, cudaEnableDefault, &qres) != cudaSuccess || !ptr) return nullptr;
    fn = reinterpret_cast<PFN_encodeTiled>(ptr);
    return fn;
}
static PFN_encodeTiled get_encode() { return get_tensor_map_encoder(); }

struct BlockTcPlan {
    CUtensorMap tm_in, tm_w, tm_o[4];
    TcParams p;
    dim3 grid;
    size_t smem_bytes;
    int dtype, ks, stride, tile;
    int halfk = 0;
    int tiles = 0;
    bool grid_final = false;
    TcLaunchOpts opts;
    void* dwp = nullptr;
    float2* pw_affine = nullptr;
    float* head_w = nullptr;
    std::string name;
};

static void plan_env_knobs(BlockPlanIn& q) {
    const char* a = getenv("FD_TC_MAX_NCTA");
    const char* d = getenv("FD_TC_CLUSTER");
    if (d && *d) q.cluster = atoi(d);
    { const char* m = getenv("FD_TC_CLUSTER_MULTIWAVE"); q.cluster_multiwave = (m && *m == '1') ? 1 : 0; }
    q.max_n_cta = a ? atoi(a) : 0;
}

static int pick_tile(const StageGeom& g) {
    return (g.h_out <= 8 && g.w_out <= 8) ? 1 : 0;
}

bool block_tc_supported(int dtype, const StageGeom& g, bool head_fused) {
    if (dtype != FD_F16 && dtype != FD_BF16) return false;
    if (!((g.ksize == 3 && (g.stride == 1 || g.stride == 2)) || (g.ksize == 5 && g.stride == 1))) return false;
    if (g.c_in % 8 || g.c_out % 8) return false;
    if (head_fused && g.c_out > 64) return false;
    return get_encode() != nullptr;
}

template <typename T, int KS, int STRIDE, int NI, int TH, int TW, bool RELU6, bool HALFK = false, int CLM = 0>
static int launch_inst2(BlockTcPlan* bp, cudaStream_t st) {
    auto kern = block_tc_kernel<T, KS, STRIDE, NI, TH, TW, RELU6, HALFK, CLM>;
    constexpr bool CL = CLM != 0;
    const int csize = CLM == 1 ? bp->p.cs : bp->p.wmc;
    const int units = CLM == 1 ? bp->tiles : bp->p.items / (bp->p.wmc > 0 ? bp->p.wmc : 1);
    static PerDeviceOnce attr_set;
    int dev = -1;
    FD_CUDA_OK(cudaGetDevice(&dev));
    if (attr_set.need(dev)) {
        FD_CUDA_OK(cudaFuncSetAttribute(kern, cudaFuncAttributeMaxDynamicSharedMemorySize, 227 * 1024));
        attr_set.done(dev);
    }
    cudaLaunchConfig_t cfg{};
    cfg.gridDim = bp->grid; cfg.blockDim = dim3(CLM == 1 ? TC_THREADS_CL : TC_THREADS); cfg.dynamicSmemBytes = bp->smem_bytes; cfg.stream = st;
    cudaLaunchAttribute attr[2];
    int na = 0;
    if (CL) {
        attr[na].id = cudaLaunchAttributeClusterDimension;
        attr[na].val.clusterDim.x = (unsigned)csize; attr[na].val.clusterDim.y = 1; attr[na].val.clusterDim.z = 1;
        ++na;
    }
    if (CL && !bp->grid_final) {
        cfg.attrs = attr; cfg.numAttrs = (unsigned)na;
        cfg.gridDim = dim3((unsigned)(units * csize), 1, 1);
        int n_cl = 0;
        FD_CUDA_OK(cudaOccupancyMaxActiveClusters(&n_cl, kern, &cfg));
        if (n_cl < 1) return fail(FD_ERR_UNSUPPORTED, "cluster-mode block kernel: no cluster of this shape fits the device");
        if (n_cl > units) n_cl = units;
        bp->grid = dim3((unsigned)(n_cl * csize), 1, 1);
        bp->grid_final = true;
        cfg.gridDim = bp->grid;
    }
    if (bp->opts.pdl) {
        attr[na].id = cudaLaunchAttributeProgrammaticStreamSerialization;
        attr[na].val.programmaticStreamSerializationAllowed = 1;
        ++na;
    }
    cfg.attrs = attr; cfg.numAttrs = (unsigned)na;
    FD_CUDA_OK(cudaLaunchKernelEx(&cfg, kern, bp->tm_in, bp->tm_w, bp->tm_o[0], bp->tm_o[1], bp->tm_o[2], bp->tm_o[3], bp->p));
    FD_CUDA_OK(cudaGetLastError());
    return FD_OK;
}
template <typename T, int KS, int STRIDE, int NI, int TH, int TW, bool HALFK = false>
static int launch_inst(BlockTcPlan* bp, cudaStream_t st) {
    if constexpr (!HALFK) {
        if (bp->p.cs > 1)
            return bp->p.act == FD_ACT_RELU6 ? launch_inst2<T, KS, STRIDE, NI, TH, TW, true, false, 1>(bp, st)
                                             : launch_inst2<T, KS, STRIDE, NI, TH, TW, false, false, 1>(bp, st);
        if (bp->p.wmc > 1)
            return bp->p.act == FD_ACT_RELU6 ? launch_inst2<T, KS, STRIDE, NI, TH, TW, true, false, 2>(bp, st)
                                             : launch_inst2<T, KS, STRIDE, NI, TH, TW, false, false, 2>(bp, st);
    }
    return bp->p.act == FD_ACT_RELU6 ? launch_inst2<T, KS, STRIDE, NI, TH, TW, true, HALFK>(bp, st)
                                     : launch_inst2<T, KS, STRIDE, NI, TH, TW, false, HALFK>(bp, st);
}

template <typename T>
static int launch_t(BlockTcPlan* bp, cudaStream_t st) {
    const int key = bp->halfk * 1000 + bp->ks * 100 + bp->stride * 10 + bp->tile;
    switch (key) {
        case 1310: return launch_inst<T, 3, 1, 1, 8, 16, true>(bp, st);
        case 310: return launch_inst<T, 3, 1, 1, 8, 16>(bp, st);
        case 311: return launch_inst<T, 3, 1, 2, 8, 8>(bp, st);
        case 320: return launch_inst<T, 3, 2, 1, 8, 16>(bp, st);
        case 321: return launch_inst<T, 3, 2, 2, 8, 8>(bp, st);
        case 510: return launch_inst<T, 5, 1, 1, 8, 16>(bp, st);
        case 511: return launch_inst<T, 5, 1, 2, 8, 8>(bp, st);
        default: return fail(FD_ERR_UNSUPPORTED, "no fused kernel instance for this block");
    }
}

int block_tc_launch(BlockTcPlan* bp, cudaStream_t st, void* head_out) {
    if (bp->p.head) {
        if (!head_out) return fail(FD_ERR_INVALID, "head-fused block needs the output pointer");
        bp->p.head_out = head_out;
    }
    return bp->dtype == FD_F16 ? launch_t<__half>(bp, st) : launch_t<__nv_bfloat16>(bp, st);
}

const char* block_tc_name(BlockTcPlan* bp) { return bp->name.c_str(); }

BlockPlanOut block_tc_debug_plan(int ksize, int stride, int h_out, int w_out, int n, int c_in, int c_out, int head) {
    StageGeom g{};
    g.h_out = h_out; g.w_out = w_out;
    BlockPlanIn q{};
    q.ksize = ksize; q.stride = stride; q.tile = pick_tile(g); q.c_in = c_in; q.c_out = c_out; q.head = head;
    const int NI = q.tile ? 2 : 1, TW = q.tile ? 8 : 16;
    q.n_tiles = ((w_out + TW - 1) / TW) * ((h_out + 7) / 8) * ((n + NI - 1) / NI);
    q.barrier_bytes = (int)sizeof(TcBarriers); q.n_sms = 132;
    q.cluster = 0;
    { const char* e = getenv("FD_TC_DW_TEAMS"); q.even_rings = (e && *e == '1') ? 0 : ((e && *e == '2') ? 1 : 2); }
    if (q.even_rings == 2 && ksize == 5 && (c_in + TC_KBLK - 1) / TC_KBLK <= 2) q.even_rings = 1;
    plan_env_knobs(q);
    return plan_block(q);
}

int block_tc_trace(BlockTcPlan* bp, cudaStream_t st, void* head_out, unsigned long long* out_host, int* rows, int* cols) {
    unsigned long long* dev = nullptr;
    const size_t bytes = 12 * TC_TRACE_N * sizeof(unsigned long long);
    FD_CUDA_OK(cudaMalloc(&dev, bytes));
    FD_CUDA_OK(cudaMemsetAsync(dev, 0, bytes, st));
    bp->p.trace = dev;
    int rc = block_tc_launch(bp, st, head_out);
    bp->p.trace = nullptr;
    if (rc == FD_OK && cudaStreamSynchronize(st) != cudaSuccess) rc = fail(FD_ERR_CUDA, "trace run failed");
    if (rc == FD_OK) cudaMemcpy(out_host, dev, bytes, cudaMemcpyDeviceToHost);
    cudaFree(dev);
    *rows = 12; *cols = TC_TRACE_N;
    return rc;
}

void block_tc_destroy(BlockTcPlan* bp) {
    if (!bp) return;
    cudaFree(bp->dwp); cudaFree(bp->pw_affine); cudaFree(bp->head_w);
    delete bp;
}

template <typename T>
__global__ void pack_dwp_kernel(const float* __restrict__ w, const float* __restrict__ scale, const float* __restrict__ bias,
                                uint8_t* __restrict__ dst, int taps, int c_in, int kblocks, int block_bytes, float post) {
    const int i = blockIdx.x * blockDim.x + threadIdx.x;
    if (i >= kblocks * 64) return;
    const int kb = i / 64, cl = i % 64, c = kb * 64 + cl;
    uint8_t* blk = dst + (size_t)kb * block_bytes;
    for (int t = 0; t < taps; ++t) {
        const T v = Traits<T>::from_f(c < c_in ? w[t * c_in + c] : 0.f);
        if (taps == 25) {
            float* row = reinterpret_cast<float*>(blk) + ((t / 5) * 32 + (cl >> 1)) * 12;
            row[(t % 5) * 2 + (cl & 1)] = Traits<T>::to_f(v);
            if (t % 5 == 0) row[10 + (cl & 1)] = 0.f;
        } else {
            reinterpret_cast<T*>(blk)[t * 64 + cl] = v;
        }
    }
    const int tb = taps == 25 ? dw_taps_bytes(5) : dw_taps_bytes(3);
    reinterpret_cast<float*>(blk + tb)[cl] = c < c_in ? scale[c] * post : 0.f;
    reinterpret_cast<float*>(blk + tb + 256)[cl] = c < c_in ? bias[c] * post : 0.f;
}
__global__ void pack_affine_kernel(const float* __restrict__ scale, const float* __restrict__ bias, float2* __restrict__ dst,
                                   int n_src, int n_dst, float post) {
    const int i = blockIdx.x * blockDim.x + threadIdx.x;
    if (i < n_dst) {
        const int pair = i >> 1, odd = i & 1;
        float* d = reinterpret_cast<float*>(dst) + pair * 4;
        d[odd] = i < n_src ? scale[i] * post : 0.f;
        d[2 + odd] = i < n_src ? bias[i] * post : 0.f;
    }
}
__global__ void pad_copy_kernel(const float* __restrict__ src, float* __restrict__ dst, int n_src, int n_dst) {
    const int i = blockIdx.x * blockDim.x + threadIdx.x;
    if (i < n_dst) dst[i] = i < n_src ? src[i] : 0.f;
}

static int padded_copy(const float* src, int n_src, int n_dst, float** out) {
    FD_CUDA_OK(cudaMalloc(out, (size_t)n_dst * 4));
    pad_copy_kernel<<<(n_dst + 255) / 256, 256>>>(src, *out, n_src, n_dst);
    FD_CUDA_OK(cudaGetLastError());
    return FD_OK;
}

static int block_wmc_auto(const StageGeom& g, const BlockPlanOut& po, int n_tiles) {
    (void)g; (void)po; (void)n_tiles;
    return 1;
}

int block_tc_prepare(int dtype, const BlockArgs& a, const float* head_w, float head_scale, float head_bias, int head_act,
                     void* head_out, bool tma_epilogue, const TcLaunchOpts& opts, BlockTcPlan** out) {
    PFN_encodeTiled encode = get_encode();
    if (!encode) return fail(FD_ERR_CUDA, "cuTensorMapEncodeTiled is not available from this driver");
    const StageGeom& g = a.g;
    BlockTcPlan* bp = new (std::nothrow) BlockTcPlan();
    if (!bp) return fail(FD_ERR_CUDA, "out of host memory");
    bp->dtype = dtype; bp->ks = g.ksize; bp->stride = g.stride; bp->tile = pick_tile(g);
    bp->opts = opts;
    {
        const char* e = getenv("FD_TC_NO_HALFK");
        bp->halfk = (g.c_in <= 32 && g.ksize == 3 && g.stride == 1 && bp->tile == 0 && !(e && *e == '1')) ? 1 : 0;
    }
    const int NI = bp->tile ? 2 : 1, TH = 8, TW = bp->tile ? 8 : 16;
    const int IH = (TH - 1) * g.stride + g.ksize, IW = (TW - 1) * g.stride + g.ksize;
    TcParams& p = bp->p;
    memset(&p, 0, sizeof(p));
    p.n = g.n; p.h_in = g.h_in; p.w_in = g.w_in; p.h_out = g.h_out; p.w_out = g.w_out; p.c_in = g.c_in; p.c_out = g.c_out;
    p.tiles_x = (g.w_out + TW - 1) / TW; p.tiles_y = (g.h_out + TH - 1) / TH;
    const int tiles_img = (g.n + NI - 1) / NI;
    const int n_tiles = p.tiles_x * p.tiles_y * tiles_img;
    p.kblocks = (g.c_in + TC_KBLK - 1) / TC_KBLK; p.cin_pad = p.kblocks * TC_KBLK;
    p.act = g.act; p.upsample = g.upsample;
    p.head = head_w != nullptr; p.head_act = head_act; p.head_scale = head_scale; p.head_bias = head_bias;
    p.skip = a.skip; p.out = a.out; p.head_out = head_out;
    p.out_pitch = g.out_pitch > 0 ? g.out_pitch : g.c_out; p.skip_pitch = g.skip_pitch > 0 ? g.skip_pitch : g.c_out;
    const int in_pitch = g.in_pitch > 0 ? g.in_pitch : g.c_in;

    BlockPlanIn pin{};
    pin.ksize = g.ksize; pin.stride = g.stride; pin.tile = bp->tile; pin.c_in = g.c_in; pin.c_out = g.c_out; pin.n_tiles = n_tiles;
    pin.head = p.head; pin.barrier_bytes = (int)sizeof(TcBarriers); pin.n_sms = opts.n_sms;
    pin.cluster = (opts.cluster && !bp->halfk) ? 0 : 1;
    { const char* e = getenv("FD_TC_DW_TEAMS"); pin.even_rings = (e && *e == '1') ? 0 : ((e && *e == '2') ? 1 : 2); }
    if (pin.even_rings == 2 && g.ksize == 5 && (g.c_in + TC_KBLK - 1) / TC_KBLK <= 2) pin.even_rings = 1;
    plan_env_knobs(pin);
    if (bp->halfk) pin.cluster = 1;
    const BlockPlanOut po = plan_block(pin);
    if (!po.ok) { delete bp; return fail(FD_ERR_UNSUPPORTED, "fused block does not fit shared memory"); }
    const int splits = po.splits;
    p.n_cta = po.n_cta; p.splits = po.splits; p.items = po.items;
    p.in_stage_bytes = po.in_stage_bytes; p.dwp_bytes = po.dwp_bytes; p.in_stage_stride = po.in_stage_stride; p.cpad_all = po.cpad_all;
    p.s_a = po.s_a; p.n_stg = po.n_stg; p.s_in = po.s_in; p.s_b = po.s_b; p.bn = po.bn; p.nb = po.nb;
    p.b_resident = po.b_resident; p.b_stage_bytes = po.b_stage_bytes;
    p.cs = po.cs; bp->tiles = n_tiles;
    { const char* e = getenv("FD_TC_EPI_HIGH"); p.epi_high = (e && *e) ? atoi(e) : 0; }
    p.dw_teams = po.dw_teams;
    p.wmc = 1;
    {
        const char* e = getenv("FD_TC_WMC");
        int want = e && *e ? atoi(e) : 0;
        if (!opts.cluster || bp->halfk) want = 1;
        if (want == 0) want = block_wmc_auto(g, po, n_tiles);
        while (want > 1 && !(p.cs == 1 && !p.b_resident && n_tiles % want == 0 && p.bn % (8 * want) == 0 && n_tiles / want >= 1)) want >>= 1;
        p.wmc = want < 1 ? 1 : want;
    }
    bp->smem_bytes = (size_t)po.smem_bytes;
    const int taps = g.ksize * g.ksize;
    (void)splits;
    const int sms = opts.n_sms;
    p.sleep_ns = opts.sleep_ns;
    {
        const char* a = getenv("FD_TC_MMA_SLEEP"); const char* b = getenv("FD_TC_DW_SLEEP");
        p.mma_sleep_ns = a ? atoi(a) : 0;
        p.dw_sleep_ns = b ? atoi(b) : 0;
    }
    bp->grid = dim3((unsigned)(p.items < sms ? p.items : sms), 1, 1);
    if (p.cs > 1) {
        int n_cl = sms / p.cs; if (n_cl > n_tiles) n_cl = n_tiles; if (n_cl < 1) n_cl = 1;
        bp->grid = dim3((unsigned)(n_cl * p.cs), 1, 1);
    } else if (p.wmc > 1) {
        int n_cl = sms / p.wmc; if (n_cl > p.items / p.wmc) n_cl = p.items / p.wmc; if (n_cl < 1) n_cl = 1;
        bp->grid = dim3((unsigned)(n_cl * p.wmc), 1, 1);
    }

    int rc = FD_OK;
    const float post = 1.0f;
    auto magic = [](int d) { return (unsigned long long)((1ULL << 40) / (unsigned long long)d) + 1ULL; };
    p.mg_splits = magic(p.splits); p.mg_tx = magic(p.tiles_x); p.mg_ty = magic(p.tiles_y);
    if (cudaMalloc(&bp->dwp, (size_t)p.kblocks * p.dwp_bytes) != cudaSuccess) rc = fail(FD_ERR_CUDA, "cudaMalloc failed");
    if (rc == FD_OK) {
        const int tot = p.kblocks * 64;
        if (dtype == FD_F16) pack_dwp_kernel<__half><<<(tot + 127) / 128, 128>>>(a.dw_w, a.dw_scale, a.dw_bias, (uint8_t*)bp->dwp, taps, g.c_in, p.kblocks, p.dwp_bytes, post);
        else pack_dwp_kernel<__nv_bfloat16><<<(tot + 127) / 128, 128>>>(a.dw_w, a.dw_scale, a.dw_bias, (uint8_t*)bp->dwp, taps, g.c_in, p.kblocks, p.dwp_bytes, post);
        if (cudaGetLastError() != cudaSuccess) rc = fail(FD_ERR_CUDA, "pack_dwp_kernel launch failed");
    }
    if (rc == FD_OK && cudaMalloc(&bp->pw_affine, (size_t)p.cpad_all * sizeof(float2)) != cudaSuccess) rc = fail(FD_ERR_CUDA, "cudaMalloc failed");
    if (rc == FD_OK) {
        pack_affine_kernel<<<(p.cpad_all + 127) / 128, 128>>>(a.pw_scale, a.pw_bias, bp->pw_affine, g.c_out, p.cpad_all, post);
        if (cudaGetLastError() != cudaSuccess) rc = fail(FD_ERR_CUDA, "pack_affine_kernel launch failed");
    }
    if (rc == FD_OK) rc = padded_copy(p.head ? head_w : a.pw_scale, p.head ? g.c_out : 0, p.cpad_all, &bp->head_w);
    if (rc == FD_OK && cudaDeviceSynchronize() != cudaSuccess) rc = fail(FD_ERR_CUDA, "parameter packing failed");
    if (rc != FD_OK) { block_tc_destroy(bp); return rc; }
    p.dwp = bp->dwp; p.pw_affine = bp->pw_affine; p.head_w = bp->head_w;

    const size_t es = 2;
    const CUtensorMapDataType dt = dtype == FD_F16 ? CU_TENSOR_MAP_DATA_TYPE_FLOAT16 : CU_TENSOR_MAP_DATA_TYPE_BFLOAT16;
    {
        cuuint64_t dims[4] = {(cuuint64_t)g.c_in, (cuuint64_t)g.w_in, (cuuint64_t)g.h_in, (cuuint64_t)g.n};
        cuuint64_t strides[3] = {(cuuint64_t)in_pitch * es, (cuuint64_t)g.w_in * in_pitch * es, (cuuint64_t)g.h_in * g.w_in * in_pitch * es};
        cuuint32_t box[4] = {(cuuint32_t)TC_KBLK, (cuuint32_t)IW, (cuuint32_t)IH, (cuuint32_t)NI};
        cuuint32_t estr[4] = {1, 1, 1, 1};
        CUresult r = encode(&bp->tm_in, dt, 4, const_cast<void*>(a.in), dims, strides, box, estr, CU_TENSOR_MAP_INTERLEAVE_NONE,
                            CU_TENSOR_MAP_SWIZZLE_NONE, CU_TENSOR_MAP_L2_PROMOTION_L2_128B, CU_TENSOR_MAP_FLOAT_OOB_FILL_NONE);
        if (r != CUDA_SUCCESS) { block_tc_destroy(bp); return fail(FD_ERR_CUDA, "cuTensorMapEncodeTiled(input) failed: " + std::to_string((int)r)); }
    }
    {
        cuuint64_t dims[2] = {(cuuint64_t)g.c_in, (cuuint64_t)g.c_out};
        cuuint64_t strides[1] = {(cuuint64_t)g.c_in * es};
        cuuint32_t box[2] = {(cuuint32_t)TC_KBLK, (cuuint32_t)(p.bn / p.wmc)};
        cuuint32_t estr[2] = {1, 1};
        CUresult r = encode(&bp->tm_w, dt, 2, const_cast<void*>(a.pw_w), dims, strides, box, estr, CU_TENSOR_MAP_INTERLEAVE_NONE,
                            CU_TENSOR_MAP_SWIZZLE_128B, CU_TENSOR_MAP_L2_PROMOTION_L2_256B, CU_TENSOR_MAP_FLOAT_OOB_FILL_NONE);
        if (r != CUDA_SUCCESS) { block_tc_destroy(bp); return fail(FD_ERR_CUDA, "cuTensorMapEncodeTiled(weights) failed: " + std::to_string((int)r)); }
    }
    memset(bp->tm_o, 0, sizeof(bp->tm_o));
    p.epi_tma = (!p.head && tma_epilogue) ? 1 : 0;
    p.epi_red = (p.epi_tma && a.skip != nullptr) ? 1 : 0;
    if (p.epi_red && (a.skip != a.out || p.skip_pitch != p.out_pitch)) { block_tc_destroy(bp); return fail(FD_ERR_STATE, "in-place skip accumulation needs out == skip"); }
    if (p.epi_tma) {
        const int up = g.upsample ? 2 : 1;
        const cuuint64_t C = (cuuint64_t)g.c_out, P = (cuuint64_t)p.out_pitch, W2 = (cuuint64_t)g.w_out * up, H2 = (cuuint64_t)g.h_out * up;
        for (int d = 0; d < (g.upsample ? 4 : 1); ++d) {
            char* base = reinterpret_cast<char*>(a.out) + ((size_t)(d >> 1) * W2 + (d & 1)) * P * es;
            cuuint64_t dims[4] = {C, (cuuint64_t)g.w_out, (cuuint64_t)g.h_out, (cuuint64_t)g.n};
            cuuint64_t strides[3] = {up * P * es, up * W2 * P * es, H2 * W2 * P * es};
            cuuint32_t box[4] = {64, (cuuint32_t)TW, (cuuint32_t)TH, (cuuint32_t)NI};
            cuuint32_t estr[4] = {1, 1, 1, 1};
            CUresult r = encode(&bp->tm_o[d], dt, 4, base, dims, strides, box, estr, CU_TENSOR_MAP_INTERLEAVE_NONE,
                                CU_TENSOR_MAP_SWIZZLE_128B, CU_TENSOR_MAP_L2_PROMOTION_L2_128B, CU_TENSOR_MAP_FLOAT_OOB_FILL_NONE);
            if (r != CUDA_SUCCESS) { block_tc_destroy(bp); return fail(FD_ERR_CUDA, "cuTensorMapEncodeTiled(output) failed: " + std::to_string((int)r)); }
        }
    }
    char buf[160];
    char clbuf[16] = "";
    if (p.cs > 1) snprintf(clbuf, sizeof(clbuf), ",cl%d", p.cs);
    else if (p.wmc > 1) snprintf(clbuf, sizeof(clbuf), ",wmc%d", p.wmc);
    if (p.dw_teams == 2) strncat(clbuf, ",t2", sizeof(clbuf) - strlen(clbuf) - 1);
    snprintf(buf, sizeof(buf), "block_tc<k%d,s%d,%s%s%s>%s%s%s[n%dx%d,bn%d%s,kb%d,in%d,a%d,b%d,e%d]", g.ksize, g.stride, bp->tile ? "2x8x8" : "1x8x16", bp->halfk ? ",k32" : "", clbuf,
             g.upsample ? "+up2x" : "", a.skip ? (p.epi_red ? "+skip(red)" : "+skip") : "", p.head ? "+head" : (p.epi_tma ? "+tmast" : ""), p.n_cta, p.splits, p.bn,
             p.b_resident ? "r" : "", p.kblocks, p.s_in, p.s_a, p.s_b, p.head ? 0 : p.n_stg);
    bp->name = buf;
    *out = bp;
    return FD_OK;
}

}
```

Baseline: 53810.

## Add fused-role warp mode for 5x5 stride-1 blocks with single K-block

Adds a 'fused role' variant of the fused depthwise+pointwise tensor-core block kernel, used for 5x5 stride-1 stages with one K-block and narrow output (or the head). In this mode the same warps do the depthwise compute and the epilogue, with resident weights and a fixed small A ring. The planner picks it by default, and an env var can disable it. The aim is to cut the cross-warp handoff and barrier overhead for small decoder stages, at the cost of less overlap between the depthwise, MMA and epilogue phases.

New measurement: 54540 (median of 6 runs). 1.4% higher.

```diff
diff --git a/fastdepth_b200/csrc/fd_api.cu b/fastdepth_b200/csrc/fd_api.cu
--- a/fastdepth_b200/csrc/fd_api.cu
+++ b/fastdepth_b200/csrc/fd_api.cu
@@ -913,6 +913,7 @@
     const int v[16] = {q.ok, q.splits, q.n_cta, q.items, q.kblocks, q.s_in, q.s_a, q.s_b, q.bn, q.nb, q.b_resident, q.n_stg,
                        q.smem_bytes, q.in_stage_stride, q.cs, q.dw_teams};
     for (int i = 0; i < 16; ++i) out[i] = v[i];
+    if (cap > 16) out[16] = q.fr;
     return FD_OK;
 }
 
diff --git a/fastdepth_b200/csrc/fd_block_plan.h b/fastdepth_b200/csrc/fd_block_plan.h
--- a/fastdepth_b200/csrc/fd_block_plan.h
+++ b/fastdepth_b200/csrc/fd_block_plan.h
@@ -30,6 +30,7 @@
     int even_rings;
     int cluster_multiwave;
     int cluster;
+    int no_fused_role;
 };
 struct BlockPlanOut {
     int ok;
@@ -40,6 +41,7 @@
     int dw_teams;
     int cs;
     int smem_bytes;
+    int fr;
 };
 
 inline bool plan_block_smem(const BlockPlanIn& q, BlockPlanOut& p) {
@@ -94,6 +96,23 @@
     return (q.even_rings && p.cs == 1 && p.s_in >= 2 && !(p.s_in & 1) && !(p.s_a & 1) && (q.even_rings == 1 || p.kblocks == 1)) ? 2 : 1;
 }
 
+inline bool plan_block_fr(const BlockPlanIn& q, BlockPlanOut& p) {
+    const int cout_pad = (q.c_out + 15) / 16 * 16;
+    if (q.no_fused_role || q.ksize != 5 || q.stride != 1 || p.kblocks != 1 || !(cout_pad <= 64 || q.head) || q.cluster > 1) return false;
+    p.splits = 1; p.n_cta = cout_pad; p.cs = 1; p.items = q.n_tiles; p.cpad_all = cout_pad;
+    p.bn = 64; p.nb = 1; p.b_resident = 1; p.s_b = p.kblocks; p.b_stage_bytes = 64 * 128;
+    p.s_a = 2; p.n_stg = q.head ? 0 : 2;
+    const int fixed = q.barrier_bytes + kPlanAlignSlack + (q.head ? 3 : 2) * p.cpad_all * 4;
+    const int rest = p.s_a * kPlanAStage + p.s_b * p.b_stage_bytes + p.n_stg * kPlanStg + fixed;
+    int s_in = (kPlanSmemBudget - rest) / p.in_stage_stride;
+    if (s_in > kPlanMaxIn) s_in = kPlanMaxIn;
+    if (s_in < p.kblocks + 1) return false;
+    p.s_in = s_in;
+    p.smem_bytes = rest + s_in * p.in_stage_stride;
+    p.fr = 1;
+    return true;
+}
+
 inline BlockPlanOut plan_block(const BlockPlanIn& q) {
     BlockPlanOut p{};
     const long sms = q.n_sms > 0 ? q.n_sms : 132;
@@ -104,6 +123,7 @@
     p.in_stage_bytes = NI * IH * IW * 128;
     p.dwp_bytes = dw_taps_bytes(q.ksize) + 512;
     p.in_stage_stride = (p.in_stage_bytes + p.dwp_bytes + 127) / 128 * 128;
+    if (plan_block_fr(q, p)) { p.ok = 1; p.dw_teams = plan_dw_teams(q, p); return p; }
     const int cout_pad = (q.c_out + 15) / 16 * 16;
     struct Cand { long t; int sp, nc, cs; };
     Cand cands[12];
diff --git a/fastdepth_b200/csrc/fd_block_tc.cu b/fastdepth_b200/csrc/fd_block_tc.cu
--- a/fastdepth_b200/csrc/fd_block_tc.cu
+++ b/fastdepth_b200/csrc/fd_block_tc.cu
@@ -91,7 +91,7 @@
         if (p.trace != nullptr && blockIdx.x == 0 && (idx) < TC_TRACE_N) p.trace[(row) * TC_TRACE_N + (idx)] = clock64(); \
     } while (0)
 
-template <typename T, int KS, int STRIDE, int NI, int TH, int TW, bool RELU6, bool HALFK = false, int CLM = 0>
+template <typename T, int KS, int STRIDE, int NI, int TH, int TW, bool RELU6, bool HALFK = false, int CLM = 0, bool FR = false>
 __global__ void __launch_bounds__(CLM == 1 ? TC_THREADS_CL : TC_THREADS, 1)
 block_tc_kernel(const __grid_constant__ CUtensorMap tm_in, const __grid_constant__ CUtensorMap tm_w,
                 const __grid_constant__ CUtensorMap tm_o0, const __grid_constant__ CUtensorMap tm_o1,
@@ -121,6 +121,7 @@
     constexpr bool CL = CLM == 1, CW = CLM == 2;
     constexpr bool kHint = CLM != 1;
     static_assert(!(HALFK && CLM != 0), "the half-K block has one K-block and resident weights: nothing to share");
+    static_assert(!FR || (KS == 5 && STRIDE == 1 && !HALFK && CLM == 0), "fused-role mode exists for the 5x5 stride-1 block only");
     const uint32_t cs = CL ? (uint32_t)p.cs : 1u;
     const uint32_t crank = (CL || CW) ? cluster_ctarank() : 0u;
     const uint32_t wmc = CW ? (uint32_t)p.wmc : 1u;
@@ -134,7 +135,7 @@
     };
 
     if (threadIdx.x == 0) {
-        const uint32_t dw_arrivals = (uint32_t)(TC_DW_WARPS / ((CL || p.dw_teams != 2) ? 1 : 2));
+        const uint32_t dw_arrivals = (uint32_t)(TC_DW_WARPS / ((FR || CL || p.dw_teams != 2) ? 1 : 2));
         for (int i = 0; i < TC_MAX_IN; ++i) { mbar_init(smem_u32(&bars->in_full[i]), 1); mbar_init(smem_u32(&bars->in_empty[i]), dw_arrivals); }
         for (int i = 0; i < TC_MAX_A; ++i) { mbar_init(smem_u32(&bars->a_full[i]), CL ? 1u : dw_arrivals); mbar_init(smem_u32(&bars->a_empty[i]), 2u * cs); }
         for (int i = 0; i < 4; ++i) mbar_init(smem_u32(&bars->dw_done[i]), TC_DW_WARPS);
@@ -167,6 +168,242 @@
     pdl_wait_prior_grid();
     if constexpr (CLM != 0) cluster_sync_all();
     else __syncthreads();
+
+    auto dw_block = [&](const uint8_t* stage, const uint8_t* prm, const f32x2 sc, const f32x2 bi, uint8_t* a_s, const int bidx) {
+        constexpr int BPR = TW / 4, BPI = (TH / 4) * BPR;
+        constexpr int TAPS = dw_taps_bytes(KS);
+        const int ni = bidx / BPI, rem = bidx % BPI, br = rem / BPR, bc = rem % BPR;
+        const uint8_t* in_s = stage + (uint32_t)((ni * IH + br * 4 * STRIDE) * IW + bc * 4 * STRIDE) * 128u + lane * 4u;
+        if constexpr (HALFK) {
+            static_assert(KS == 3 && STRIDE == 1, "half-K depthwise exists for the 3x3 stride-1 block only");
+            const int hl = lane & 15, hh = lane >> 4;
+            const uint8_t* in_h = in_s - lane * 4 + hl * 4 + (hh * 2 * IW) * 128;
+            const f32x2 sc2 = *reinterpret_cast<const f32x2*>(prm + TAPS + hl * 8);
+            const f32x2 bi2 = *reinterpret_cast<const f32x2*>(prm + TAPS + 256 + hl * 8);
+            f32x2 acc[2][4];
+#pragma unroll
+            for (int a = 0; a < 2; ++a)
+#pragma unroll
+                for (int b = 0; b < 4; ++b) acc[a][b] = 0ull;
+            f32x2 wq[KS][KS];
+#pragma unroll
+            for (int iy = 0; iy < 1 + KS; ++iy) {
+                if (iy < KS) {
+#pragma unroll
+                    for (int kx = 0; kx < KS; ++kx)
+                        wq[iy][kx] = MF::widen(*reinterpret_cast<const uint32_t*>(prm + (iy * KS + kx) * 128 + hl * 4));
+                }
+                f32x2 row[IBW];
+#pragma unroll
+                for (int ix = 0; ix < IBW; ++ix) row[ix] = MF::widen(*reinterpret_cast<const uint32_t*>(in_h + (iy * IW + ix) * 128));
+#pragma unroll
+                for (int oy = 0; oy < 2; ++oy) {
+                    const int ky = iy - oy;
+                    if (ky < 0 || ky >= KS) continue;
+#pragma unroll
+                    for (int ox = 0; ox < 4; ++ox)
+#pragma unroll
+                        for (int kx = 0; kx < KS; ++kx) ffma2(acc[oy][ox], row[ox + kx], wq[ky][kx]);
+                    if (ky == KS - 1) {
+#pragma unroll
+                        for (int ox = 0; ox < 4; ++ox) {
+                            const int m = (ni * TH + br * 4 + hh * 2 + oy) * TW + bc * 4 + ox;
+                            *reinterpret_cast<uint32_t*>(a_s + m * 128 + (((hl >> 2) ^ (m & 7)) << 4) + ((hl & 3) << 2)) =
+                                MF::template pack_act<RELU6>(ffma2_abc(acc[oy][ox], sc2, bi2));
+                        }
+                    }
+                }
+            }
+        } else {
+            f32x2 acc[4][4];
+#pragma unroll
+            for (int a = 0; a < 4; ++a)
+#pragma unroll
+                for (int b = 0; b < 4; ++b) acc[a][b] = 0ull;
+            constexpr bool kTapsInRegs = KS == 3;
+            f32x2 wq[kTapsInRegs ? KS : 1][KS];
+#pragma unroll
+            for (int iy = 0; iy < IBH; ++iy) {
+                if constexpr (kTapsInRegs) {
+                    if (iy < KS) {
+#pragma unroll
+                        for (int kx = 0; kx < KS; ++kx)
+                            wq[iy][kx] = MF::widen(*reinterpret_cast<const uint32_t*>(prm + (iy * KS + kx) * 128 + lane * 4));
+                    }
+                }
+                f32x2 row[IBW];
+#pragma unroll
+                for (int ix = 0; ix < IBW; ++ix) row[ix] = MF::widen(*reinterpret_cast<const uint32_t*>(in_s + (iy * IW + ix) * 128));
+#pragma unroll
+                for (int oy = 0; oy < 4; ++oy) {
+                    const int ky = iy - oy * STRIDE;
+                    if (ky < 0 || ky >= KS) continue;
+                    f32x2 wk[KS];
+                    if constexpr (kTapsInRegs) {
+#pragma unroll
+                        for (int kx = 0; kx < KS; ++kx) wk[kx] = wq[ky][kx];
+                    } else {
+                        const uint8_t* tr = prm + (ky * 32 + lane) * 48;
+                        const uint4 t01 = lds_u4_here(tr), t23 = lds_u4_here(tr + 16), t4 = lds_u4_here(tr + 32);
+                        wk[0] = ((f32x2)t01.y << 32) | t01.x; wk[1] = ((f32x2)t01.w << 32) | t01.z;
+                        wk[2] = ((f32x2)t23.y << 32) | t23.x; wk[3] = ((f32x2)t23.w << 32) | t23.z;
+                        wk[4] = ((f32x2)t4.y << 32) | t4.x;
+                    }
+#pragma unroll
+                    for (int ox = 0; ox < 4; ++ox)
+#pragma unroll
+                        for (int kx = 0; kx < KS; ++kx) ffma2(acc[oy][ox], row[ox * STRIDE + kx], wk[kx]);
+                    if (ky == KS - 1) {
+#pragma unroll
+                        for (int ox = 0; ox < 4; ++ox) {
+                            const int m = (ni * TH + br * 4 + oy) * TW + bc * 4 + ox;
+                            *reinterpret_cast<uint32_t*>(a_s + m * 128 + (((lane >> 2) ^ (m & 7)) << 4) + ((lane & 3) << 2)) =
+                                MF::template pack_act<RELU6>(ffma2_abc(acc[oy][ox], sc, bi));
+                        }
+                    }
+                }
+            }
+        }
+    };
+
+    auto epilogue = [&](auto& acc, const ItemCoord& c, const int r0, const int cq, const int ew, const bool elected, const uint32_t bar_id,
+                        uint8_t* stg0, const int n_stg, uint32_t& stg_flip, const int tr) {
+        constexpr int NCH = sizeof(acc) / sizeof(acc[0]);
+        constexpr uint32_t bar_n = 256u;
+        const int nch = (p.n_cta + 63) >> 6;
+        T* __restrict__ outp = reinterpret_cast<T*>(p.out);
+        const T* __restrict__ skipp = reinterpret_cast<const T*>(p.skip);
+    if (!p.head) {
+        const float2* aff = s_pw_affine + c.n0;
+#pragma unroll
+        for (int cb = 0; cb < NCH; ++cb) {
+            if (cb >= nch) break;
+            uint8_t* stg = stg0 + (n_stg == 2 ? (stg_flip & 1u) * 16384u : 0u);
+            ++stg_flip;
+            if (n_stg == 1 && stg_flip > 1) {
+                if (p.epi_tma && elected) bulk_wait_read0();
+                asm volatile("bar.sync %0, %1;" ::"r"(bar_id), "r"(bar_n) : "memory");
+            }
+#pragma unroll
+            for (int i = 0; i < 8; ++i) {
+                if (cb * 64 + i * 8 < p.n_cta) {
+                    const float4 af = *reinterpret_cast<const float4*>(aff + cb * 64 + i * 8 + cq);
+                    const f32x2 sc = f32x2_make(af.x, af.y), bi = f32x2_make(af.z, af.w);
+#pragma unroll
+                    for (int h = 0; h < 2; ++h) {
+                        const int r = r0 + 8 * h;
+                        *reinterpret_cast<uint32_t*>(stg + r * 128 + ((i ^ (r & 7)) << 4) + cq * 2) =
+                            MF::template pack_act<RELU6>(ffma2_abc(f32x2_make(acc[cb][4 * i + 2 * h], acc[cb][4 * i + 2 * h + 1]), sc, bi));
+                    }
+                }
+            }
+            if (p.epi_tma) {
+                fence_proxy_async();
+                if (elected && cb == 0) TC_TRACE(9, tr);
+                if (elected) bulk_wait_read0();
+                asm volatile("bar.sync %0, %1;" ::"r"(bar_id), "r"(bar_n) : "memory");
+                if (elected && cb == 0) TC_TRACE(10, tr);
+                if (elected) {
+                    const uint32_t src = smem_u32(stg);
+                    const int cc = c.n0 + cb * 64;
+                    if (!p.upsample) {
+                        tma_store_4d(&tm_o0, src, cc, c.ox0, c.oy0, c.img0);
+                    } else if (!p.epi_red) {
+                        tma_store_4d(&tm_o0, src, cc, c.ox0, c.oy0, c.img0);
+                        tma_store_4d(&tm_o1, src, cc, c.ox0, c.oy0, c.img0);
+                        tma_store_4d(&tm_o2, src, cc, c.ox0, c.oy0, c.img0);
+                        tma_store_4d(&tm_o3, src, cc, c.ox0, c.oy0, c.img0);
+                    } else {
+                        tma_reduce_add_4d(&tm_o0, src, cc, c.ox0, c.oy0, c.img0);
+                        tma_reduce_add_4d(&tm_o1, src, cc, c.ox0, c.oy0, c.img0);
+                        tma_reduce_add_4d(&tm_o2, src, cc, c.ox0, c.oy0, c.img0);
+                        tma_reduce_add_4d(&tm_o3, src, cc, c.ox0, c.oy0, c.img0);
+                    }
+                    bulk_commit_group();
+                    if (cb == 0) TC_TRACE(11, tr);
+                }
+                continue;
+            }
+            asm volatile("bar.sync %0, %1;" ::"r"(bar_id), "r"(bar_n) : "memory");
+            const int et = ew * 32 + lane;
+            const int ch = et & 7;
+            const int ccol = cb * 64 + ch * 8;
+            const bool cok = ccol < p.n_cta && c.n0 + ccol + 8 <= p.c_out;
+#pragma unroll
+            for (int k = 0; k < 4; ++k) {
+                const int rr = (et >> 3) + 32 * k;
+                const int r_ni = rr / (TH * TW), r_ty = (rr / TW) % TH, r_tx = rr % TW;
+                const int pimg = c.img0 + r_ni, poy = c.oy0 + r_ty, pox = c.ox0 + r_tx;
+                if (!(cok && pimg < p.n && poy < p.h_out && pox < p.w_out)) continue;
+                const uint4 v = *reinterpret_cast<const uint4*>(stg + rr * 128 + ((ch ^ (rr & 7)) << 4));
+                if (!p.upsample) {
+                    *reinterpret_cast<uint4*>(outp + (((size_t)pimg * p.h_out + poy) * p.w_out + pox) * p.out_pitch + c.n0 + ccol) = v;
+                } else {
+                    const int w2 = 2 * p.w_out;
+                    const size_t pix00 = ((size_t)pimg * 2 * p.h_out + 2 * poy) * w2 + 2 * pox;
+                    size_t off[4], soff[4];
+#pragma unroll
+                    for (int d = 0; d < 4; ++d) {
+                        const size_t pix = pix00 + (size_t)(d >> 1) * w2 + (d & 1);
+                        off[d] = pix * p.out_pitch + c.n0 + ccol;
+                        soff[d] = pix * p.skip_pitch + c.n0 + ccol;
+                    }
+                    if (skipp != nullptr) {
+                        uint4 sv[4];
+#pragma unroll
+                        for (int d = 0; d < 4; ++d) sv[d] = __ldg(reinterpret_cast<const uint4*>(skipp + soff[d]));
+                        const uint32_t vv[4] = {v.x, v.y, v.z, v.w};
+#pragma unroll
+                        for (int d = 0; d < 4; ++d) {
+                            const uint32_t sk[4] = {sv[d].x, sv[d].y, sv[d].z, sv[d].w};
+                            uint32_t z[4];
+#pragma unroll
+                            for (int j = 0; j < 4; ++j) {
+                                const float2 a = MF::unpack(vv[j]), bq = MF::unpack(sk[j]);
+                                z[j] = MF::pack(a.x + bq.x, a.y + bq.y);
+                            }
+                            *reinterpret_cast<uint4*>(outp + off[d]) = make_uint4(z[0], z[1], z[2], z[3]);
+                        }
+                    } else {
+#pragma unroll
+                        for (int d = 0; d < 4; ++d) *reinterpret_cast<uint4*>(outp + off[d]) = v;
+                    }
+                }
+            }
+        }
+    } else {
+        float dot[2][2] = {{0.f, 0.f}, {0.f, 0.f}};
+#pragma unroll
+        for (int i = 0; i < 8; ++i) {
+            const int c0 = i * 8 + cq;
+            if (i * 8 < p.n_cta) {
+                const float4 af = *reinterpret_cast<const float4*>(s_pw_affine + c0);
+                const f32x2 sc = f32x2_make(af.x, af.y), bi = f32x2_make(af.z, af.w);
+                const uint32_t hw = s_head_w2[c0 >> 1];
+#pragma unroll
+                for (int h = 0; h < 2; ++h) {
+                    const uint32_t hv = MF::template pack_act<RELU6>(ffma2_abc(f32x2_make(acc[0][4 * i + 2 * h], acc[0][4 * i + 2 * h + 1]), sc, bi));
+                    MF::fma2(dot[h][0], dot[h][1], hv, hw);
+                }
+            }
+        }
+#pragma unroll
+        for (int h = 0; h < 2; ++h) {
+            float d = dot[h][0] + dot[h][1];
+            d += __shfl_xor_sync(0xffffffffu, d, 1);
+            d += __shfl_xor_sync(0xffffffffu, d, 2);
+            const int r = r0 + 8 * h;
+            const int img = c.img0 + r / (TH * TW), oy = c.oy0 + (r / TW) % TH, ox = c.ox0 + r % TW;
+            if ((lane & 3) == 0 && img < p.n && oy < p.h_out && ox < p.w_out) {
+                const float y = apply_act(fmaf(d, p.head_scale, p.head_bias), p.head_act);
+                const uint32_t yy = MF::pack(y, y);
+                T* ho = reinterpret_cast<T*>(p.head_out) + ((size_t)img * 2 * p.h_out + 2 * oy) * (2 * p.w_out) + 2 * ox;
+                *reinterpret_cast<uint32_t*>(ho) = yy;
+                *reinterpret_cast<uint32_t*>(ho + 2 * p.w_out) = yy;
+            }
+        }
+    }
+    };
 
     if (warp == TC_WARP_TMA) {
         if (lane == 0) {
@@ -231,8 +468,56 @@
                         if (peer != crank) bulk_copy_to_peer(mapa_u32(slot, peer), slot, (uint32_t)TC_A_STAGE_BYTES, mapa_u32(bar, peer));
                 }
         }
+    } else if constexpr (FR) {
+        const int g = warp >> 2, wq = warp & 3, pair = g >> 1, h = g & 1;
+        const int ew = h * 4 + wq;
+        const int r0 = h * 64 + wq * 16 + (lane >> 2), cq = (lane & 3) * 2;
+        const bool elected = ew == 0 && lane == 0;
+        const uint32_t pair_bar = 1u + (uint32_t)pair, wg_bar = 3u + (uint32_t)g;
+        uint8_t* a_s = smem + a_off + (uint32_t)g * 8192u - (uint32_t)h * 8192u;
+        const uint32_t a_lo = sw128_desc_lo(smem_base + a_off + (uint32_t)g * 8192u), b_lo0 = sw128_desc_lo(smem_base + b_off);
+        Ring rin;
+        int tr = 0;
+        uint32_t stg_flip = 0;
+        bool first = true;
+        const bool tracer = warp == 0 && lane == 0;
+        mbar_wait_sel<kHint>(smem_u32(&bars->aff_full), 0);
+        int j = 0;
+        for (int u = u_first; u < u_count; u += u_stride, ++j) {
+            if ((j & 1) != pair) { rin.next((uint32_t)p.s_in); continue; }
+            const ItemCoord c = decode_item(p, u, NI, TH, TW);
+            const uint32_t s = rin.s, ph = rin.ph;
+            rin.next((uint32_t)p.s_in);
+            mbar_wait_sleep_sel<kHint>(smem_u32(&bars->in_full[s]), ph, (uint32_t)p.dw_sleep_ns);
+            if (tracer) TC_TRACE(1, tr);
+            const uint8_t* stage = smem + in_off + s * p.in_stage_stride;
+            const uint8_t* prm = stage + p.in_stage_bytes;
+            constexpr int TAPS = dw_taps_bytes(KS);
+            const f32x2 sc = *reinterpret_cast<const f32x2*>(prm + TAPS + lane * 8);
+            const f32x2 bi = *reinterpret_cast<const f32x2*>(prm + TAPS + 256 + lane * 8);
+            dw_block(stage, prm, sc, bi, a_s, h * 4 + wq);
+            if (tracer) TC_TRACE(2, tr);
+            __syncwarp();
+            if (lane == 0) mbar_arrive(smem_u32(&bars->in_empty[s]));
+            fence_proxy_async();
+            asm volatile("bar.sync %0, 128;" ::"r"(wg_bar) : "memory");
+            if (first) mbar_wait_sel<kHint>(smem_u32(&bars->b_full[0]), 0);
+            first = false;
+            float acc[1][32];
+#pragma unroll
+            for (int i = 0; i < 32; ++i) acc[0][i] = 0.f;
+            wgmma_fence();
+#pragma unroll
+            for (int k4 = 0; k4 < 4; ++k4)
+                wgmma_n64<T>(acc[0], sw128_desc(a_lo + 2u * k4), sw128_desc(b_lo0 + 2u * k4), k4 > 0 ? 1u : 0u);
+            wgmma_commit();
+            wgmma_wait0();
+            if (tracer) { TC_TRACE(5, tr); ++tr; }
+            epilogue(acc, c, r0, cq, ew, elected, pair_bar, smem + stg_off + (uint32_t)pair * 16384u, 1, stg_flip, tr);
+            if (tracer) TC_TRACE(7, tr);
+        }
+        if (p.epi_tma && elected) bulk_wait_all();
     } else if (rwarp >= TC_WARP_DW0 && rwarp < TC_WARP_DW0 + TC_DW_WARPS) {
-        constexpr int BPR = TW / 4, BPI = (TH / 4) * BPR;
         const int dwi = rwarp - TC_WARP_DW0;
         const int teams = CL ? 1 : p.dw_teams;
         const int team = teams == 2 ? dwi >> 2 : 0, member = teams == 2 ? dwi & 3 : dwi, nblk = teams;
@@ -259,101 +544,7 @@
                 mbar_wait_sel<kHint>(smem_u32(&bars->a_empty[sa]), pha ^ 1u);
                 uint8_t* a_s = smem + a_off + sa * TC_A_STAGE_BYTES;
 #pragma unroll 1
-                for (int blk = 0; blk < nblk; ++blk) {
-                const int bidx = member * nblk + blk;
-                const int ni = bidx / BPI, rem = bidx % BPI, br = rem / BPR, bc = rem % BPR;
-                const uint8_t* in_s = stage + (uint32_t)((ni * IH + br * 4 * STRIDE) * IW + bc * 4 * STRIDE) * 128u + lane * 4u;
-                if constexpr (HALFK) {
-                    static_assert(KS == 3 && STRIDE == 1, "half-K depthwise exists for the 3x3 stride-1 block only");
-                    const int hl = lane & 15, hh = lane >> 4;
-                    const uint8_t* in_h = in_s - lane * 4 + hl * 4 + (hh * 2 * IW) * 128;
-                    const f32x2 sc2 = *reinterpret_cast<const f32x2*>(prm + TAPS + hl * 8);
-                    const f32x2 bi2 = *reinterpret_cast<const f32x2*>(prm + TAPS + 256 + hl * 8);
-                    f32x2 acc[2][4];
-#pragma unroll
-                    for (int a = 0; a < 2; ++a)
-#pragma unroll
-                        for (int b = 0; b < 4; ++b) acc[a][b] = 0ull;
-                    f32x2 wq[KS][KS];
-#pragma unroll
-                    for (int iy = 0; iy < 1 + KS; ++iy) {
-                        if (iy < KS) {
-#pragma unroll
-                            for (int kx = 0; kx < KS; ++kx)
-                                wq[iy][kx] = MF::widen(*reinterpret_cast<const uint32_t*>(prm + (iy * KS + kx) * 128 + hl * 4));
-                        }
-                        f32x2 row[IBW];
-#pragma unroll
-                        for (int ix = 0; ix < IBW; ++ix) row[ix] = MF::widen(*reinterpret_cast<const uint32_t*>(in_h + (iy * IW + ix) * 128));
-#pragma unroll
-                        for (int oy = 0; oy < 2; ++oy) {
-                            const int ky = iy - oy;
-                            if (ky < 0 || ky >= KS) continue;
-#pragma unroll
-                            for (int ox = 0; ox < 4; ++ox)
-#pragma unroll
-                                for (int kx = 0; kx < KS; ++kx) ffma2(acc[oy][ox], row[ox + kx], wq[ky][kx]);
-                            if (ky == KS - 1) {
-#pragma unroll
-                                for (int ox = 0; ox < 4; ++ox) {
-                                    const int m = (ni * TH + br * 4 + hh * 2 + oy) * TW + bc * 4 + ox;
-                                    *reinterpret_cast<uint32_t*>(a_s + m * 128 + (((hl >> 2) ^ (m & 7)) << 4) + ((hl & 3) << 2)) =
-                                        MF::template pack_act<RELU6>(ffma2_abc(acc[oy][ox], sc2, bi2));
-                                }
-                            }
-                        }
-                    }
-                } else {
-                    f32x2 acc[4][4];
-#pragma unroll
-                    for (int a = 0; a < 4; ++a)
-#pragma unroll
-                        for (int b = 0; b < 4; ++b) acc[a][b] = 0ull;
-                    constexpr bool kTapsInRegs = KS == 3;
-                    f32x2 wq[kTapsInRegs ? KS : 1][KS];
-#pragma unroll
-                    for (int iy = 0; iy < IBH; ++iy) {
-                        if constexpr (kTapsInRegs) {
-                            if (iy < KS) {
-#pragma unroll
-                                for (int kx = 0; kx < KS; ++kx)
-                                    wq[iy][kx] = MF::widen(*reinterpret_cast<const uint32_t*>(prm + (iy * KS + kx) * 128 + lane * 4));
-                            }
-                        }
-                        f32x2 row[IBW];
-#pragma unroll
-                        for (int ix = 0; ix < IBW; ++ix) row[ix] = MF::widen(*reinterpret_cast<const uint32_t*>(in_s + (iy * IW + ix) * 128));
-#pragma unroll
-                        for (int oy = 0; oy < 4; ++oy) {
-                            const int ky = iy - oy * STRIDE;
-                            if (ky < 0 || ky >= KS) continue;
-                            f32x2 wk[KS];
-                            if constexpr (kTapsInRegs) {
-#pragma unroll
-                                for (int kx = 0; kx < KS; ++kx) wk[kx] = wq[ky][kx];
-                            } else {
-                                const uint8_t* tr = prm + (ky * 32 + lane) * 48;
-                                const uint4 t01 = lds_u4_here(tr), t23 = lds_u4_here(tr + 16), t4 = lds_u4_here(tr + 32);
-                                wk[0] = ((f32x2)t01.y << 32) | t01.x; wk[1] = ((f32x2)t01.w << 32) | t01.z;
-                                wk[2] = ((f32x2)t23.y << 32) | t23.x; wk[3] = ((f32x2)t23.w << 32) | t23.z;
-                                wk[4] = ((f32x2)t4.y << 32) | t4.x;
-                            }
-#pragma unroll
-                            for (int ox = 0; ox < 4; ++ox)
-#pragma unroll
-                                for (int kx = 0; kx < KS; ++kx) ffma2(acc[oy][ox], row[ox * STRIDE + kx], wk[kx]);
-                            if (ky == KS - 1) {
-#pragma unroll
-                                for (int ox = 0; ox < 4; ++ox) {
-                                    const int m = (ni * TH + br * 4 + oy) * TW + bc * 4 + ox;
-                                    *reinterpret_cast<uint32_t*>(a_s + m * 128 + (((lane >> 2) ^ (m & 7)) << 4) + ((lane & 3) << 2)) =
-                                        MF::template pack_act<RELU6>(ffma2_abc(acc[oy][ox], sc, bi));
-                                }
-                            }
-                        }
-                    }
-                }
-                }
+                for (int blk = 0; blk < nblk; ++blk) dw_block(stage, prm, sc, bi, a_s, member * nblk + blk);
                 if (tracer) TC_TRACE(2, tr);
                 __syncwarp();
                 if (lane == 0) mbar_arrive(smem_u32(&bars->in_empty[s]));
@@ -370,9 +561,7 @@
         const int r0 = wg * 64 + wq * 16 + (lane >> 2), cq = (lane & 3) * 2;
         const bool leader = wq == 0 && lane == 0;
         const bool elected = ew == 0 && lane == 0;
-        constexpr uint32_t bar_id = 1u, bar_n = 256u;
-        T* __restrict__ outp = reinterpret_cast<T*>(p.out);
-        const T* __restrict__ skipp = reinterpret_cast<const T*>(p.skip);
+        constexpr uint32_t bar_id = 1u;
         const int n_stg = p.n_stg < 2 ? 1 : 2;
         const int nch = (p.n_cta + 63) >> 6;
         const int bn_ch = p.bn >> 6;
@@ -453,136 +642,7 @@
                 if (elected) { TC_TRACE(5, tr); ++tr; }
             }
 
-            if (!p.head) {
-                const float2* aff = s_pw_affine + c.n0;
-#pragma unroll
-                for (int cb = 0; cb < TC_NCH; ++cb) {
-                    if (cb >= nch) break;
-                    uint8_t* stg = smem + stg_off + (n_stg == 2 ? (stg_flip & 1u) * 16384u : 0u);
-                    ++stg_flip;
-                    if (n_stg == 1 && stg_flip > 1) {
-                        if (p.epi_tma && elected) bulk_wait_read0();
-                        asm volatile("bar.sync %0, %1;" ::"r"(bar_id), "r"(bar_n) : "memory");
-                    }
-#pragma unroll
-                    for (int i = 0; i < 8; ++i) {
-                        if (cb * 64 + i * 8 < p.n_cta) {
-                            const float4 af = *reinterpret_cast<const float4*>(aff + cb * 64 + i * 8 + cq);
-                            const f32x2 sc = f32x2_make(af.x, af.y), bi = f32x2_make(af.z, af.w);
-#pragma unroll
-                            for (int h = 0; h < 2; ++h) {
-                                const int r = r0 + 8 * h;
-                                *reinterpret_cast<uint32_t*>(stg + r * 128 + ((i ^ (r & 7)) << 4) + cq * 2) =
-                                    MF::template pack_act<RELU6>(ffma2_abc(f32x2_make(acc[cb][4 * i + 2 * h], acc[cb][4 * i + 2 * h + 1]), sc, bi));
-                            }
-                        }
-                    }
-                    if (p.epi_tma) {
-                        fence_proxy_async();
-                        if (elected && cb == 0) TC_TRACE(9, tr);
-                        if (elected) bulk_wait_read0();
-                        asm volatile("bar.sync %0, %1;" ::"r"(bar_id), "r"(bar_n) : "memory");
-                        if (elected && cb == 0) TC_TRACE(10, tr);
-                        if (elected) {
-                            const uint32_t src = smem_u32(stg);
-                            const int cc = c.n0 + cb * 64;
-                            if (!p.upsample) {
-                                tma_store_4d(&tm_o0, src, cc, c.ox0, c.oy0, c.img0);
-                            } else if (!p.epi_red) {
-                                tma_store_4d(&tm_o0, src, cc, c.ox0, c.oy0, c.img0);
-                                tma_store_4d(&tm_o1, src, cc, c.ox0, c.oy0, c.img0);
-                                tma_store_4d(&tm_o2, src, cc, c.ox0, c.oy0, c.img0);
-                                tma_store_4d(&tm_o3, src, cc, c.ox0, c.oy0, c.img0);
-                            } else {
-                                tma_reduce_add_4d(&tm_o0, src, cc, c.ox0, c.oy0, c.img0);
-                                tma_reduce_add_4d(&tm_o1, src, cc, c.ox0, c.oy0, c.img0);
-                                tma_reduce_add_4d(&tm_o2, src, cc, c.ox0, c.oy0, c.img0);
-                                tma_reduce_add_4d(&tm_o3, src, cc, c.ox0, c.oy0, c.img0);
-                            }
-                            bulk_commit_group();
-                            if (cb == 0) TC_TRACE(11, tr);
-                        }
-                        continue;
-                    }
-                    asm volatile("bar.sync %0, %1;" ::"r"(bar_id), "r"(bar_n) : "memory");
-                    const int et = ew * 32 + lane;
-                    const int ch = et & 7;
-                    const int ccol = cb * 64 + ch * 8;
-                    const bool cok = ccol < p.n_cta && c.n0 + ccol + 8 <= p.c_out;
-#pragma unroll
-                    for (int k = 0; k < 4; ++k) {
-                        const int rr = (et >> 3) + 32 * k;
-                        const int r_ni = rr / (TH * TW), r_ty = (rr / TW) % TH, r_tx = rr % TW;
-                        const int pimg = c.img0 + r_ni, poy = c.oy0 + r_ty, pox = c.ox0 + r_tx;
-                        if (!(cok && pimg < p.n && poy < p.h_out && pox < p.w_out)) continue;
-                        const uint4 v = *reinterpret_cast<const uint4*>(stg + rr * 128 + ((ch ^ (rr & 7)) << 4));
-                        if (!p.upsample) {
-                            *reinterpret_cast<uint4*>(outp + (((size_t)pimg * p.h_out + poy) * p.w_out + pox) * p.out_pitch + c.n0 + ccol) = v;
-                        } else {
-                            const int w2 = 2 * p.w_out;
-                            const size_t pix00 = ((size_t)pimg * 2 * p.h_out + 2 * poy) * w2 + 2 * pox;
-                            size_t off[4], soff[4];
-#pragma unroll
-                            for (int d = 0; d < 4; ++d) {
-                                const size_t pix = pix00 + (size_t)(d >> 1) * w2 + (d & 1);
-                                off[d] = pix * p.out_pitch + c.n0 + ccol;
-                                soff[d] = pix * p.skip_pitch + c.n0 + ccol;
-                            }
-                            if (skipp != nullptr) {
-                                uint4 sv[4];
-#pragma unroll
-                                for (int d = 0; d < 4; ++d) sv[d] = __ldg(reinterpret_cast<const uint4*>(skipp + soff[d]));
-                                const uint32_t vv[4] = {v.x, v.y, v.z, v.w};
-#pragma unroll
-                                for (int d = 0; d < 4; ++d) {
-                                    const uint32_t sk[4] = {sv[d].x, sv[d].y, sv[d].z, sv[d].w};
-                                    uint32_t z[4];
-#pragma unroll
-                                    for (int j = 0; j < 4; ++j) {
-                                        const float2 a = MF::unpack(vv[j]), bq = MF::unpack(sk[j]);
-                                        z[j] = MF::pack(a.x + bq.x, a.y + bq.y);
-                                    }
-                                    *reinterpret_cast<uint4*>(outp + off[d]) = make_uint4(z[0], z[1], z[2], z[3]);
-                                }
-                            } else {
-#pragma unroll
-                                for (int d = 0; d < 4; ++d) *reinterpret_cast<uint4*>(outp + off[d]) = v;
-                            }
-                        }
-                    }
-                }
-            } else {
-                float dot[2][2] = {{0.f, 0.f}, {0.f, 0.f}};
-#pragma unroll
-                for (int i = 0; i < 8; ++i) {
-                    const int c0 = i * 8 + cq;
-                    if (i * 8 < p.n_cta) {
-                        const float4 af = *reinterpret_cast<const float4*>(s_pw_affine + c0);
-                        const f32x2 sc = f32x2_make(af.x, af.y), bi = f32x2_make(af.z, af.w);
-                        const uint32_t hw = s_head_w2[c0 >> 1];
-#pragma unroll
-                        for (int h = 0; h < 2; ++h) {
-                            const uint32_t hv = MF::template pack_act<RELU6>(ffma2_abc(f32x2_make(acc[0][4 * i + 2 * h], acc[0][4 * i + 2 * h + 1]), sc, bi));
-                            MF::fma2(dot[h][0], dot[h][1], hv, hw);
-                        }
-                    }
-                }
-#pragma unroll
-                for (int h = 0; h < 2; ++h) {
-                    float d = dot[h][0] + dot[h][1];
-                    d += __shfl_xor_sync(0xffffffffu, d, 1);
-                    d += __shfl_xor_sync(0xffffffffu, d, 2);
-                    const int r = r0 + 8 * h;
-                    const int img = c.img0 + r / (TH * TW), oy = c.oy0 + (r / TW) % TH, ox = c.ox0 + r % TW;
-                    if ((lane & 3) == 0 && img < p.n && oy < p.h_out && ox < p.w_out) {
-                        const float y = apply_act(fmaf(d, p.head_scale, p.head_bias), p.head_act);
-                        const uint32_t yy = MF::pack(y, y);
-                        T* ho = reinterpret_cast<T*>(p.head_out) + ((size_t)img * 2 * p.h_out + 2 * oy) * (2 * p.w_out) + 2 * ox;
-                        *reinterpret_cast<uint32_t*>(ho) = yy;
-                        *reinterpret_cast<uint32_t*>(ho + 2 * p.w_out) = yy;
-                    }
-                }
-            }
+            epilogue(acc, c, r0, cq, ew, elected, bar_id, smem + stg_off, n_stg, stg_flip, tr);
             if (elected) TC_TRACE(7, tr);
         }
         if (p.epi_tma && elected) bulk_wait_all();
@@ -609,6 +669,7 @@
     size_t smem_bytes;
     int dtype, ks, stride, tile;
     int halfk = 0;
+    int fr = 0;
     int tiles = 0;
     bool grid_final = false;
     TcLaunchOpts opts;
@@ -623,6 +684,7 @@
     const char* d = getenv("FD_TC_CLUSTER");
     if (d && *d) q.cluster = atoi(d);
     { const char* m = getenv("FD_TC_CLUSTER_MULTIWAVE"); q.cluster_multiwave = (m && *m == '1') ? 1 : 0; }
+    { const char* f = getenv("FD_TC_FUSED_ROLE"); q.no_fused_role = (f && *f == '0') ? 1 : 0; }
     q.max_n_cta = a ? atoi(a) : 0;
 }
 
@@ -638,9 +700,9 @@
     return get_encode() != nullptr;
 }
 
-template <typename T, int KS, int STRIDE, int NI, int TH, int TW, bool RELU6, bool HALFK = false, int CLM = 0>
+template <typename T, int KS, int STRIDE, int NI, int TH, int TW, bool RELU6, bool HALFK = false, int CLM = 0, bool FR = false>
 static int launch_inst2(BlockTcPlan* bp, cudaStream_t st) {
-    auto kern = block_tc_kernel<T, KS, STRIDE, NI, TH, TW, RELU6, HALFK, CLM>;
+    auto kern = block_tc_kernel<T, KS, STRIDE, NI, TH, TW, RELU6, HALFK, CLM, FR>;
     constexpr bool CL = CLM != 0;
     const int csize = CLM == 1 ? bp->p.cs : bp->p.wmc;
     const int units = CLM == 1 ? bp->tiles : bp->p.items / (bp->p.wmc > 0 ? bp->p.wmc : 1);
@@ -683,6 +745,11 @@
 }
 template <typename T, int KS, int STRIDE, int NI, int TH, int TW, bool HALFK = false>
 static int launch_inst(BlockTcPlan* bp, cudaStream_t st) {
+    if constexpr (KS == 5 && STRIDE == 1) {
+        if (bp->fr)
+            return bp->p.act == FD_ACT_RELU6 ? launch_inst2<T, KS, STRIDE, NI, TH, TW, true, false, 0, true>(bp, st)
+                                             : launch_inst2<T, KS, STRIDE, NI, TH, TW, false, false, 0, true>(bp, st);
+    }
     if constexpr (!HALFK) {
         if (bp->p.cs > 1)
             return bp->p.act == FD_ACT_RELU6 ? launch_inst2<T, KS, STRIDE, NI, TH, TW, true, false, 1>(bp, st)
@@ -847,7 +914,7 @@
     p.in_stage_bytes = po.in_stage_bytes; p.dwp_bytes = po.dwp_bytes; p.in_stage_stride = po.in_stage_stride; p.cpad_all = po.cpad_all;
     p.s_a = po.s_a; p.n_stg = po.n_stg; p.s_in = po.s_in; p.s_b = po.s_b; p.bn = po.bn; p.nb = po.nb;
     p.b_resident = po.b_resident; p.b_stage_bytes = po.b_stage_bytes;
-    p.cs = po.cs; bp->tiles = n_tiles;
+    p.cs = po.cs; bp->tiles = n_tiles; bp->fr = po.fr;
     { const char* e = getenv("FD_TC_EPI_HIGH"); p.epi_high = (e && *e) ? atoi(e) : 0; }
     p.dw_teams = po.dw_teams;
     p.wmc = 1;
@@ -941,7 +1008,8 @@
     char clbuf[16] = "";
     if (p.cs > 1) snprintf(clbuf, sizeof(clbuf), ",cl%d", p.cs);
     else if (p.wmc > 1) snprintf(clbuf, sizeof(clbuf), ",wmc%d", p.wmc);
-    if (p.dw_teams == 2) strncat(clbuf, ",t2", sizeof(clbuf) - strlen(clbuf) - 1);
+    if (bp->fr) strncat(clbuf, ",fr", sizeof(clbuf) - strlen(clbuf) - 1);
+    else if (p.dw_teams == 2) strncat(clbuf, ",t2", sizeof(clbuf) - strlen(clbuf) - 1);
     snprintf(buf, sizeof(buf), "block_tc<k%d,s%d,%s%s%s>%s%s%s[n%dx%d,bn%d%s,kb%d,in%d,a%d,b%d,e%d]", g.ksize, g.stride, bp->tile ? "2x8x8" : "1x8x16", bp->halfk ? ",k32" : "", clbuf,
              g.upsample ? "+up2x" : "", a.skip ? (p.epi_red ? "+skip(red)" : "+skip") : "", p.head ? "+head" : (p.epi_tma ? "+tmast" : ""), p.n_cta, p.splits, p.bn,
              p.b_resident ? "r" : "", p.kblocks, p.s_in, p.s_a, p.s_b, p.head ? 0 : p.n_stg);
```
